# YaoTiancheng/DirectComputeRayTracing

Measured on AMD Instinct MI355X. Metric: Mrays/s and ms/spp at 1920x1080, 8-bounce wavefront, higher is better.
Workload: dtype f32; 1 GPU; cornell_box_obj 1920x1080, 1733 spp (1 spp/step, film stripes across 1 GPU(s)), 8 bounces, wavefront, point light; spp=1733, max_bounce=8, streams_per_gpu=3, snapshot_spp=1733, parallelism=single GPU, 3 concurrent pipelines per GPU (cost-balanced bands), partition=balanced, interleave=False, bands_per_rank=3, rays=48252902736

## Files before the change

### directcomputeraytracing_amd/_abi.py

```python
from __future__ import annotations

import ctypes as C
import os
from pathlib import Path

PKG_DIR = Path(__file__).resolve().parent
LIB_PATH = PKG_DIR / "libdcrt.so"

DCRT_OK = 0
ABI_VERSION = 4
ERRORS = {-1: "DCRT_E_INVALID_ARG", -2: "DCRT_E_HIP", -3: "DCRT_E_NO_SCENE", -4: "DCRT_E_IO",
          -5: "DCRT_E_LIMIT", -6: "DCRT_E_NO_DEVICE"}
LIGHT_INDEX_INVALID = 0xFFFFFFFF
FEATURE_GGX_SAMPLE_VNDF = 0x01
FEATURE_NO_FRONT_TO_BACK = 0x02
FEATURE_LIGHT_VISIBLE = 0x04
FEATURE_WATERTIGHT = 0x08
FEATURE_ALLOW_ANYHIT = 0x10
FEATURE_DEFAULT = FEATURE_GGX_SAMPLE_VNDF | FEATURE_LIGHT_VISIBLE | FEATURE_WATERTIGHT
FILTER_BOX, FILTER_TRIANGLE, FILTER_GAUSSIAN, FILTER_MITCHELL, FILTER_LANCZOS = range(5)
MATERIAL_DIFFUSE, MATERIAL_PLASTIC, MATERIAL_CONDUCTOR, MATERIAL_DIELECTRIC, MATERIAL_THIN_DIELECTRIC = range(5)
MAX_LIGHT_COUNT = 5000
DIRTY_LIGHTS = 0x01
DIRTY_MATERIALS = 0x02
DIRTY_INSTANCE_FLAGS = 0x04
DIRTY_CAMERA = 0x08
DIRTY_SCENE = 0x10
(OUTPUT_PATH_TRACING, OUTPUT_SHADING_NORMAL, OUTPUT_SHADING_TANGENT, OUTPUT_ALBEDO, OUTPUT_NEGATIVE_NDOTV,
 OUTPUT_BACKFACE, OUTPUT_ITERATION_COUNT) = range(7)


class Vertex(C.Structure):
    _fields_ = [("position", C.c_float * 3), ("normal", C.c_float * 3), ("tangent", C.c_float * 3),
                ("texcoord", C.c_float * 2)]


class BVHNode(C.Structure):
    _fields_ = [("bbox_min", C.c_float * 3), ("bbox_max", C.c_float * 3), ("right_child_or_prim_index", C.c_uint32),
                ("misc", C.c_uint32)]


class Material(C.Structure):
    _fields_ = [("albedo", C.c_float * 3), ("albedo_texture_index", C.c_int32), ("ior", C.c_float * 3),
# ... 91 lines not shown


class AdaptiveReport(C.Structure):
    _fields_ = [("images", C.c_uint32), ("check_points", C.c_uint32), ("pixel_samples", C.c_uint64),
                ("active_blocks", C.c_uint32), ("total_blocks", C.c_uint32)]


class RayStats(C.Structure):
    _fields_ = [("extension_rays", C.c_uint64), ("shadow_rays", C.c_uint64), ("new_paths", C.c_uint64),
                ("iterations", C.c_uint64), ("images_completed", C.c_uint64)]


class FilmPartition(C.Structure):
    _fields_ = [("world_size", C.c_uint32), ("rank", C.c_uint32), ("stripe_height", C.c_uint32),
                ("halo_rows", C.c_uint32)]


class TraversalStats(C.Structure):
    _fields_ = [("ext_node_visits", C.c_uint64), ("ext_triangle_tests", C.c_uint64), ("ext_blas_entries", C.c_uint64),
                ("shadow_node_visits", C.c_uint64), ("shadow_triangle_tests", C.c_uint64),
                ("shadow_blas_entries", C.c_uint64), ("ext_launches", C.c_uint64), ("ext_kernel_ms", C.c_double),
                ("ext_max_node_visits", C.c_uint64), ("shadow_max_node_visits", C.c_uint64),
                ("material_launches", C.c_uint64), ("material_kernel_ms", C.c_double),
                ("control_launches", C.c_uint64), ("control_kernel_ms", C.c_double)]


class TracerInfo(C.Structure):
    _fields_ = [("path_pool_size", C.c_uint32), ("scene_in_lds", C.c_uint32), ("cached_nodes", C.c_uint32),
                ("cached_triangles", C.c_uint32), ("cast_block", C.c_uint32), ("traversal_stack", C.c_uint32),
                ("material_generic", C.c_uint32), ("pair_traversal", C.c_uint32), ("control_grid", C.c_uint32),
                ("material_grid", C.c_uint32), ("cast_grid", C.c_uint32), ("material_lds", C.c_uint32),
                ("cast_identity", C.c_uint32), ("stack_lds_rows", C.c_uint32), ("ring_rows", C.c_uint32),
                ("cast_waves_per_cu", C.c_uint32), ("shadow_cells", C.c_uint32), ("shadow_cell_max_leaves", C.c_uint32),
                ("shadow_cell_mean_leaves", C.c_float), ("shadow_inline", C.c_uint32)]


class ShadowCellsInfo(C.Structure):
    _fields_ = [("resolution", C.c_uint32), ("leaf_count", C.c_uint32), ("node_count", C.c_uint32),
                ("max_leaves", C.c_uint32), ("mean_leaves", C.c_float), ("r0", C.c_float)]


class UploadStats(C.Structure):
    _fields_ = [("scene_uploads", C.c_uint64), ("material_updates", C.c_uint64), ("light_updates", C.c_uint64),
                ("instance_flag_updates", C.c_uint64), ("geometry_bytes", C.c_uint64), ("shading_bytes", C.c_uint64),
                ("graph_invalidations", C.c_uint64)]


class MaterialSetting(C.Structure):
    _fields_ = [("albedo", C.c_float * 3), ("roughness", C.c_float), ("ior", C.c_float * 3), ("opacity", C.c_float),
                ("k", C.c_float * 3), ("tiling", C.c_float * 2), ("material_type", C.c_uint32),
                ("albedo_texture_index", C.c_int32), ("opacity_texture_index", C.c_int32),
                ("internal_scattering_mode", C.c_uint32), ("multiscattering", C.c_uint32),
                ("is_two_sided", C.c_uint32), ("has_roughness_texture", C.c_uint32)]


class SceneSettings(C.Structure):
    _fields_ = [("resolution", C.c_uint32 * 2), ("max_bounce_count", C.c_uint32), ("camera_type", C.c_uint32),
                ("fov_x", C.c_float), ("focal_length", C.c_float), ("focal_distance", C.c_float),
                ("relative_aperture", C.c_float), ("aperture_blade_count", C.c_uint32), ("aperture_rotation", C.c_float),
                ("film_size", C.c_float * 2), ("camera_position", C.c_float * 3), ("camera_euler_angles", C.c_float * 3),
                ("features", C.c_uint32), ("has_environment_light", C.c_uint32), ("environment_color", C.c_float * 3),
                ("env_cube_rgb", C.POINTER(C.c_float)), ("env_cube_size", C.c_uint32),
                ("mesh_light_count", C.c_uint32), ("punctual_light_count", C.c_uint32),
                ("material_count", C.c_uint32), ("texture_count", C.c_uint32)]


class ObjMesh(C.Structure):
# ... 123 lines not shown
    ("dcrt_tracer_render_guides", _I, [_P, _U, _U]),
    ("dcrt_tracer_guide_device_ptrs", _I, [_P, C.POINTER(_P), C.POINTER(_P)]),
    ("dcrt_tracer_read_guides", _I, [_P, _FP, _FP]),
    ("dcrt_tracer_denoise", _I, [_P, C.POINTER(DenoiseParams)]),
    ("dcrt_tracer_denoise_device", _I, [_P, C.POINTER(DenoiseParams), _U, _U, _P, _P, _P, _P]),
    ("dcrt_tracer_denoise_images", _I, [_P, C.POINTER(DenoiseParams), _U, _U, _FP, _FP, _FP, _FP]),
    ("dcrt_tracer_read_denoised", _I, [_P, _FP]),
    ("dcrt_tracer_denoised_device_ptr", _I, [_P, C.POINTER(_P)]),
    ("dcrt_tracer_resolve_denoised", _I, [_P, C.POINTER(PostFxParams), C.POINTER(C.c_uint8), _FP]),
    ("dcrt_tracer_denoise_timings", _I, [_P, _FP, _U, C.POINTER(C.c_uint32)]),
    ("dcrt_tracer_set_convergence", _I, [_P, _I]),
    ("dcrt_tracer_film_image_count", _I, [_P, C.POINTER(C.c_uint32)]),
    ("dcrt_tracer_half_film_device_ptr", _I, [_P, C.POINTER(_P)]),
    ("dcrt_tracer_read_half_film", _I, [_P, _FP]),
    ("dcrt_tracer_add_half_film_device", _I, [_P, _P]),
    ("dcrt_tracer_noise", _I, [_P, C.c_float, C.POINTER(NoiseStats)]),
    ("dcrt_tracer_noise_device", _I, [_P, _U, _U, _P, _P, C.c_float, _P, _P, C.POINTER(NoiseStats)]),
    ("dcrt_tracer_film_pass_timing", _I, [_P, C.POINTER(C.c_uint64), C.POINTER(C.c_double)]),
    ("dcrt_tracer_noise_map_device_ptrs", _I, [_P, C.POINTER(_P), C.POINTER(_P)]),
    ("dcrt_tracer_read_noise_maps", _I, [_P, _FP, _FP]),
    ("dcrt_tracer_render_converged", _I, [_P, _U, C.POINTER(ConvergeParams), C.POINTER(FilterParams), C.POINTER(NoiseStats),
                                          C.POINTER(C.c_int)]),
    ("dcrt_tracer_set_adaptive", _I, [_P, _I]),
    ("dcrt_tracer_set_sample_blocks", _I, [_P, C.POINTER(C.c_uint32), _U]),
    ("dcrt_tracer_get_sample_blocks", _I, [_P, C.POINTER(C.c_uint32), _U, C.POINTER(C.c_uint32)]),
    ("dcrt_tracer_update_sample_blocks", _I, [_P, C.c_float, _U, C.POINTER(C.c_uint32)]),
    ("dcrt_tracer_sample_blocks_device", _I, [_P, _U, _U, _P, _P, C.c_float, _U, _P, _P, C.POINTER(C.c_uint32)]),
    ("dcrt_tracer_adaptive_timings", _I, [_P, _FP, _FP, _FP]),
    ("dcrt_tracer_render_adaptive", _I, [_P, _U, C.POINTER(ConvergeParams), _U, C.POINTER(FilterParams), C.POINTER(NoiseStats),
                                         C.POINTER(C.c_int), C.POINTER(AdaptiveReport)]),
    ("dcrt_write_bmp", _I, [C.c_char_p, _U, _U, C.POINTER(C.c_uint8)]),
    ("dcrt_device_math_eval", _I, [_P, _I, _FP, _U, _FP]),
    ("dcrt_device_bsdf_eval", _I, [_P, C.POINTER(BsdfProbeMaterial), _U, _FP, _FP, _U, _FP, _FP]),
    ("dcrt_device_bsdf_sample", _I, [_P, C.POINTER(BsdfProbeMaterial), _U, _FP, _FP, _U, _FP, _FP, _FP, C.POINTER(C.c_uint32)]),
]

_lib = None


class DCRTError(RuntimeError):
    pass


def load_library(path: os.PathLike | str | None = None):
    global _lib
    if _lib is not None:
        return _lib
    p = Path(path) if path else Path(os.environ.get("DCRT_LIB", LIB_PATH))
    if not p.exists():
        raise DCRTError(f"native library {p} is missing: run __graft_entry__.build() (no CPU fallback exists)")
    lib = C.CDLL(str(p))
    for name, res, args in SIGNATURES:
        fn = getattr(lib, name)
        fn.restype = res
        fn.argtypes = args
    if lib.dcrt_abi_version() != ABI_VERSION:
        raise DCRTError(f"{p}: ABI version {lib.dcrt_abi_version()}, this binding expects {ABI_VERSION}")
    _lib = lib
    return lib


def check(rc: int, what: str = "") -> None:
    if rc != DCRT_OK:
        lib = load_library()
        msg = lib.dcrt_last_error().decode(errors="replace")
        raise DCRTError(f"{what or 'dcrt call'} failed: {ERRORS.get(rc, rc)}: {msg}")
# ... 5 lines not shown
```

### directcomputeraytracing_amd/csrc/device/dbsdf.h

```cpp
#pragma once

#include "dscene.h"

namespace dcrt {
namespace dev {

struct LCtx { V3 H; float WOdotH; };
DEV void calc_h(V3 wo, V3 wi, LCtx& c)
{
    c.H = wi + wo;
    c.H = all_zero(c.H) ? mk(0.0f, 0.0f, 0.0f) : normalize(c.H);
    c.WOdotH = dot(c.H, wo);
}

DEV float fresnel_dielectric(float cosThetaI, float etaO, float etaI)
{
    cosThetaI = fminf(fmaxf(cosThetaI, -1.0f), 1.0f);
    if (cosThetaI < 0.0f) { const float t = etaO; etaO = etaI; etaI = t; cosThetaI = -cosThetaI; }
    const float sinThetaI = sqrtf(1.0f - cosThetaI * cosThetaI);
    const float sinThetaT = etaO / etaI * sinThetaI;
    if (sinThetaT >= 1.0f) return 1.0f;
    const float cosThetaT = sqrtf(1.0f - sinThetaT * sinThetaT);
    const float Rparl = ((etaI * cosThetaI) - (etaO * cosThetaT)) / ((etaI * cosThetaI) + (etaO * cosThetaT));
    const float Rperp = ((etaO * cosThetaI) - (etaI * cosThetaT)) / ((etaO * cosThetaI) + (etaI * cosThetaT));
// ... 184 lines not shown
DEV V3 specular_brdf_sample(V3 wo, float* value, float* pdf, LCtx& c)
{
    const V3 wi = mk(-wo.x, -wo.y, wo.z);
    c.H = mk(0.0f, 0.0f, 1.0f); c.WOdotH = wo.z;
    if (wo.z <= 0.0f) return wi;
    *value = 1.0f / wi.z;
    *pdf = 1.0f;
    return wi;
}
template <bool NO_SCALE>
DEV V3 specular_bsdf_sample(V3 wo, float sample, float etaO, float etaI, bool thin, float* value, float* pdf, LCtx& c)
{
    V3 wi = mk(0.0f, 0.0f, 0.0f);
    c.H = mk(0.0f, 0.0f, 1.0f); c.WOdotH = wo.z;
    if (etaO == etaI) { *value = 1.0f / wo.z; *pdf = 1.0f; return -wo; }
    if (wo.z == 0.0f) return wi;
    float F = fresnel_dielectric(wo.z, etaO, etaI);
    float T = 1.0f - F;
    if (thin && F < 1.0f) { F = F + T * T * F / (1.0f - F * F); T = 1.0f - F; }
    if (sample < F) {
        wi = mk(-wo.x, -wo.y, wo.z);
        *value = F / wi.z;
        *pdf = F;
    } else {
        wi = !thin ? refract(-wo, mk(0.0f, 0.0f, 1.0f), etaO / etaI) : -wo;
        if (wi.z == 0.0f) return wi;
        if (NO_SCALE) *value = T / (-wi.z);
        else *value = T * (!thin ? (etaO * etaO) / (etaI * etaI) : 1.0f) / (-wi.z);
        *pdf = T;
    }
    return wi;
}

DEV V3 isf_factor(const DeviceScene& s, float alpha, V3 albedo, float ior, uint32_t mode)
{
    if (mode == DCRT_INTERNAL_SCATTERING_IGNORE) return mk(1.0f, 1.0f, 1.0f);
    const float avg = lut_brdf_dielectric_avg(s, alpha, ior, true);
    const float f = 1.0f - avg;
    V3 factor = mk(f, f, f);
    if (mode == DCRT_INTERNAL_SCATTERING_MULTIPLE)
        factor = mk(factor.x / (1.0f - albedo.x * avg), factor.y / (1.0f - albedo.y * avg), factor.z / (1.0f - albedo.z * avg));
    return factor;
}
DEV V3 to_tbn(V3 w, V3 t, V3 b, V3 n) { return mk(dot(w, t), dot(w, b), dot(w, n)); }
DEV V3 from_tbn(V3 w, V3 t, V3 b, V3 n)
{
    return mk(w.x * t.x + w.y * b.x + w.z * n.x, w.x * t.y + w.y * b.y + w.z * n.y, w.x * t.z + w.y * b.z + w.z * n.z);
}
DEV V3 splat(float f) { return mk(f, f, f); }

struct DielectricMs { float E, Eavg, EinvAvg, ratio; };
DEV DielectricMs dielectric_ms(const DeviceScene& s, float cosThetaO, float alpha, float ior, bool inverted)
{
    const float EavgEnter = lut_bsdf_avg(s, alpha, ior, true);
    const float FavgEnter = favg_dielectric(1.0f / ior);
    const float EavgLeave = lut_bsdf_avg(s, alpha, ior, false);
    const float FavgLeave = favg_dielectric(ior);
    const float rf = reciprocal_factor(FavgLeave, FavgEnter, EavgLeave, EavgEnter, ior);
    DielectricMs d;
    d.E = lut_bsdf(s, cosThetaO, alpha, ior, inverted);
    const float Favg = inverted ? FavgEnter : FavgLeave;
    d.Eavg = inverted ? EavgEnter : EavgLeave;
    d.EinvAvg = inverted ? EavgLeave : EavgEnter;
    d.ratio = (inverted ? 1.0f - rf : rf) * (1.0f - Favg);
    return d;
}

struct BsdfFrame {
    V3 b, wo;
    bool inv;
    bool any;
    float E, Eavg;
    float diel;
    V3 isf;
    DielectricMs dms;
};
DEV BsdfFrame bsdf_frame(const DeviceScene& s, V3 woW, const Intersection& it)
{
    BsdfFrame f;
    f.b = cross(it.normal, it.tangent);
    f.wo = to_tbn(woW, it.tangent, f.b, it.normal);
    f.inv = f.wo.z < 0.0f;
    if (f.inv) f.wo.z = -f.wo.z;
    f.any = !f.inv || it.isTwoSided;
    const float cosO = f.wo.z;
    const uint32_t type = it.materialType;
    f.E = 0.0f; f.Eavg = 0.0f; f.diel = 0.0f; f.isf = mk(1.0f, 1.0f, 1.0f);
    f.dms.E = 0.0f; f.dms.Eavg = 0.0f; f.dms.EinvAvg = 0.0f; f.dms.ratio = 0.0f;
    if (it.multiscattering && (type == DCRT_MATERIAL_TYPE_PLASTIC || type == DCRT_MATERIAL_TYPE_CONDUCTOR) && f.any) {
        f.E = lut_brdf(s, cosO, it.alpha);
        f.Eavg = lut_brdf_avg(s, it.alpha);
    }
    if (type == DCRT_MATERIAL_TYPE_PLASTIC && f.any) {
        f.diel = lut_brdf_dielectric(s, cosO, it.alpha, it.ior.x, false);
        f.isf = isf_factor(s, it.alpha, it.albedo, it.ior.x, it.internalScatteringMode);
    }
    if (type == DCRT_MATERIAL_TYPE_DIELECTRIC && it.multiscattering && !(it.alpha < kAlphaThreshold))
        f.dms = dielectric_ms(s, cosO, it.alpha, it.ior.x, f.inv);
    return f;
}

DEV V3 evaluate_bsdf(const DeviceScene& s, bool vndf, V3 wiW, const BsdfFrame& f, const Intersection& it)
{
    const V3 wo = f.wo;
    V3 wi = to_tbn(wiW, it.tangent, f.b, it.normal);
    const bool inv = f.inv;
    if (inv) wi.z = -wi.z;
    LCtx c;
    calc_h(wo, wi, c);
    const bool smooth = it.alpha < kAlphaThreshold;
    V3 value = mk(0.0f, 0.0f, 0.0f);
    const uint32_t type = it.materialType;
    if (type != DCRT_MATERIAL_TYPE_DIELECTRIC && type != DCRT_MATERIAL_TYPE_THIN_DIELECTRIC) {
        bool hasL = false, hasCT = false, hasMS = false, dielF = false;
        float ratioL = 0.0f;
        const float E = f.E, Eavg = f.Eavg;
        V3 Fms = mk(0.0f, 0.0f, 0.0f), isf = mk(1.0f, 1.0f, 1.0f);
        const bool any = f.any;
        if (type == DCRT_MATERIAL_TYPE_DIFFUSE && any) {
            hasL = true; ratioL = 1.0f;
        } else if (type == DCRT_MATERIAL_TYPE_PLASTIC && any) {
            hasL = true; hasCT = !smooth; hasMS = it.multiscattering && !smooth; dielF = true;
            ratioL = 1.0f - f.diel;
            if (hasMS) {
                const float fm = ms_fresnel(Eavg, favg_dielectric(it.ior.x));
                Fms = splat(fm);
                ratioL = fmaxf(ratioL - Fms.x * (1.0f - E), 0.0f);
            }
// ... 191 lines not shown
```

### directcomputeraytracing_amd/csrc/device/dscene.h

```cpp
#pragma once

#include "../../../include/dcrt.h"
#include "dmath.h"
#include "../host/shadow_cells.h"

namespace dcrt {
namespace dev {

constexpr uint32_t kCapMatDiffuse = 1u << 0;
constexpr uint32_t kCapMatPlastic = 1u << 1;
constexpr uint32_t kCapMatConductor = 1u << 2;
constexpr uint32_t kCapMatDielectric = 1u << 3;
constexpr uint32_t kCapMatThin = 1u << 4;
constexpr uint32_t kCapMultiscatter = 1u << 5;
constexpr uint32_t kCapTextures = 1u << 6;
constexpr uint32_t kCapLightPoint = 1u << 7;
constexpr uint32_t kCapLightMesh = 1u << 8;
constexpr uint32_t kCapLightDirectional = 1u << 9;
constexpr uint32_t kCapLightEnv = 1u << 10;
constexpr uint32_t kCapEnvCube = 1u << 11;
constexpr uint32_t kCapAll = (1u << 12) - 1u;
constexpr uint32_t kCapMaterialsMask = 0x1Fu;
constexpr uint32_t kCapLightShift = 7;
constexpr uint32_t kCapOpaqueDelta = kCapMatDiffuse | kCapMatPlastic | kCapMatConductor | kCapLightPoint | kCapLightDirectional;
// ... 20 lines not shown
    const uint32_t* instanceFlags;
    const uint32_t* instanceIdentity;
    const uint32_t* overrides;
    const dcrt_material* materials;
    const dcrt_light* lights;
    const TextureDesc* textures;
    const uint8_t* texels;
    const float* srgbTable;
    const float* envCube;
    const uint16_t* lutBrdf;
    const uint16_t* lutBrdfAvg;
    const uint16_t* lutBrdfDielectric;
    const uint16_t* lutBrdfDielectricAvg;
    const uint16_t* lutBsdf;
    const uint16_t* lutBsdfAvg;
    uint32_t instanceCount;
    uint32_t nodeCount;
    uint32_t triangleCount;
    uint32_t envCubeSize;
    uint32_t stackSize;
    uint32_t stackRows;
    uint32_t ringRows;
    uint32_t* spill;
    uint32_t cachedNodes;
    uint32_t cachedTris;
    uint32_t cachedInstances;
    uint32_t singlePrimLeaves;
    uint32_t pairLayout;
    uint32_t skipRoot;
    uint32_t ldsMaterials, ldsLights;
    const uint64_t* shadowCells;
    const uint32_t* shadowLeaves;
    uint32_t shadowRes;
};

__host__ __device__ inline uint32_t material_lds_bytes(uint32_t T, uint32_t I, uint32_t M, uint32_t L)
{
    return 16u * (9u * T + 3u * I) + 4u * (2u * I + 13u * M + 7u * L);
}

__host__ __device__ inline uint32_t material_cells_lds_bytes(uint32_t nodes, uint32_t T) { return 32u * nodes + 144u * T + 4u * kCellWords; }
__host__ __device__ inline uint32_t material_cells_lds_offset(uint32_t shadingBytes) { return (shadingBytes + 15u) & ~15u; }

enum : int { kLayoutFlat = 0, kLayoutPairs = 1, kLayoutScene = 2 };
template <int LAYOUT>
DEV void node_children(const DeviceScene& sc, uint32_t node, uint32_t right, uint32_t* left, uint32_t* rightChild)
{
    const uint32_t r = right | (node & 0x80000000u);
    const bool pairs = LAYOUT == kLayoutPairs || (LAYOUT == kLayoutScene && sc.pairLayout != 0u);
    *left = pairs ? r : node + 1u;
    *rightChild = pairs ? r + 1u : r;
}


DEV float4* scene_cache(const DeviceScene& sc, uint32_t* stackMem, uint32_t shift)
{
    return (float4*)(stackMem + (sc.stackRows << shift));
}
typedef float LoadF4 __attribute__((ext_vector_type(4)));
DEV float4 lds_load4(const float4* genericLds, uint32_t i)
{
    const __attribute__((address_space(3))) LoadF4* p = (const __attribute__((address_space(3))) LoadF4*)(uint32_t)(uintptr_t)genericLds;
    const LoadF4 v = p[i];
    return make_float4(v.x, v.y, v.z, v.w);
}
DEV uint64_t global_load_u64(const uint64_t* g, size_t i)
{
// ... 657 lines not shown
    if (r > (float)(slices - 1)) return slices - 1;
    return (int)r;
}
DEV float remap(uint32_t dim, float u) { return u * ((float)(dim - 1) / (float)dim) + 0.5f / (float)dim; }
DEV float sample_array(const uint16_t* tex, uint32_t w, uint32_t h, uint32_t slices, float uu, float vv, float ww, uint32_t dz, uint32_t off)
{
    const float slicePos = ww * ((float)dz - 1.0f);
    const float fraction = slicePos - floorf(slicePos);
    const float u = remap(w, uu), v = remap(h, vv);
    const uint32_t s0 = (uint32_t)(int32_t)slicePos + off;
    const uint32_t s1 = (uint32_t)(int32_t)slicePos + 1u + off;
    const int i0 = array_slice((float)s0, (int)slices), i1 = array_slice((float)s1, (int)slices);
    const float a = bilinear_u16(tex + (size_t)i0 * w * h, (int)w, (int)h, u, v);
    const float b = bilinear_u16(tex + (size_t)i1 * w * h, (int)w, (int)h, u, v);
    return lerp(a, b, fraction);
}
DEV float lut_brdf(const DeviceScene& s, float cosThetaO, float alpha)
{
    return bilinear_u16(s.lutBrdf, 32, 32, remap(32, cosThetaO), remap(32, alpha));
}
DEV float lut_brdf_avg(const DeviceScene& s, float alpha)
{
    const float u = remap(32, alpha);
    return bilinear_u16(s.lutBrdfAvg, 32, 1, u, u);
}
DEV float lut_brdf_dielectric(const DeviceScene& s, float cosThetaO, float alpha, float eta, bool entering)
{
    return sample_array(s.lutBrdfDielectric, 32, 16, 32, cosThetaO, alpha, (eta - 1.0f) / 2.0f, 16, entering ? 16u : 0u);
}
DEV float lut_brdf_dielectric_avg(const DeviceScene& s, float alpha, float eta, bool entering)
{
    return sample_array(s.lutBrdfDielectricAvg, 16, 16, 2, alpha, (eta - 1.0f) / 2.0f, 0.0f, 1, entering ? 1u : 0u);
}
DEV float lut_bsdf(const DeviceScene& s, float cosThetaO, float alpha, float eta, bool entering)
{
    return sample_array(s.lutBsdf, 32, 16, 32, cosThetaO, alpha, (eta - 1.0f) / 2.0f, 16, entering ? 16u : 0u);
}
DEV float lut_bsdf_avg(const DeviceScene& s, float alpha, float eta, bool entering)
{
    return sample_array(s.lutBsdfAvg, 16, 16, 2, alpha, (eta - 1.0f) / 2.0f, 0.0f, 1, entering ? 1u : 0u);
}

DEV int wrapi(int i, int n) { const int r = i % n; return r < 0 ? r + n : r; }
DEV void texel(const DeviceScene& s, const TextureDesc& t, int x, int y, float* o)
{
    if (t.format == DCRT_TEXTURE_FORMAT_R8_UNORM) {
        o[0] = (float)s.texels[t.offset + (size_t)y * t.width + x] / 255.0f; o[1] = 0.0f; o[2] = 0.0f; o[3] = 1.0f;
    } else {
        const uint8_t* p = s.texels + t.offset + ((size_t)y * t.width + x) * 4;
        o[0] = s.srgbTable[p[0]]; o[1] = s.srgbTable[p[1]]; o[2] = s.srgbTable[p[2]]; o[3] = (float)p[3] / 255.0f;
    }
}
DEV void sample_texture_wrap(const DeviceScene& s, uint32_t index, float u, float v, float* out)
{
    const TextureDesc t = s.textures[index];
    if (t.width == 0 || t.height == 0) { out[0] = out[1] = out[2] = out[3] = 0.0f; return; }
    const int w = (int)t.width, h = (int)t.height;
    const float x = u * (float)w - 0.5f, y = v * (float)h - 0.5f;
    const float fx0 = floorf(x), fy0 = floorf(y);
    const float fx = x - fx0, fy = y - fy0;
    const int x0 = wrapi((int)fx0, w), x1 = wrapi((int)fx0 + 1, w);
    const int y0 = wrapi((int)fy0, h), y1 = wrapi((int)fy0 + 1, h);
    float a[4], b[4], c[4], d[4];
    texel(s, t, x0, y0, a); texel(s, t, x1, y0, b); texel(s, t, x0, y1, c); texel(s, t, x1, y1, d);
    for (int i = 0; i < 4; ++i) {
        const float top = a[i] * (1.0f - fx) + b[i] * fx;
// ... 2 lines not shown
    }
}
DEV V3 sample_env(const DeviceScene& s, V3 d)
{
    const float ax = fabsf(d.x), ay = fabsf(d.y), az = fabsf(d.z);
    int face; float sc, tc, ma;
    if (ax >= ay && ax >= az) { ma = ax; if (d.x >= 0.0f) { face = 0; sc = -d.z; tc = -d.y; } else { face = 1; sc = d.z; tc = -d.y; } }
    else if (ay >= az) { ma = ay; if (d.y >= 0.0f) { face = 2; sc = d.x; tc = d.z; } else { face = 3; sc = d.x; tc = -d.z; } }
    else { ma = az; if (d.z >= 0.0f) { face = 4; sc = d.x; tc = -d.y; } else { face = 5; sc = -d.x; tc = -d.y; } }
    const float u = (sc / ma + 1.0f) * 0.5f, v = (tc / ma + 1.0f) * 0.5f;
    const int n = (int)s.envCubeSize;
    const float x = u * (float)n - 0.5f, y = v * (float)n - 0.5f;
    const float fx0 = floorf(x), fy0 = floorf(y);
    const float fx = x - fx0, fy = y - fy0;
    const int x0 = clampi((int)fx0, 0, n - 1), x1 = clampi((int)fx0 + 1, 0, n - 1);
    const int y0 = clampi((int)fy0, 0, n - 1), y1 = clampi((int)fy0 + 1, 0, n - 1);
    const float* base = s.envCube + (size_t)face * n * n * 3;
    float o[3];
    for (int i = 0; i < 3; ++i) {
        const float a = base[((size_t)y0 * n + x0) * 3 + i], b = base[((size_t)y0 * n + x1) * 3 + i];
        const float c = base[((size_t)y1 * n + x0) * 3 + i], e = base[((size_t)y1 * n + x1) * 3 + i];
        const float top = a * (1.0f - fx) + b * fx;
        const float bot = c * (1.0f - fx) + e * fx;
        o[i] = top * (1.0f - fy) + bot * fy;
    }
    return mk(o[0], o[1], o[2]);
}

struct Intersection {
    V3 albedo; float alpha;
    V3 position, normal, tangent, geometryNormal, ior;
    bool isTwoSided, backface, multiscattering;
    uint32_t internalScatteringMode, materialType, lightIndex, triangleIndex;
};

DEV V3 bary3(V3 p0, V3 p1, V3 p2, float u, float v)
{
    V3 r1 = p1 - p0, r2 = p2 - p0;
    r1 = r1 * u; r2 = r2 * v;
    r1 = r1 + p0; r1 = r1 + r2;
    return r1;
}

template <uint32_t CAPS = kCapAll>
DEV void hit_to_intersection(const DeviceScene& s, const HitRecord& h, Intersection& it)
{
    const uint32_t inst = h.inst, tri = h.tri & 0x7FFFFFFFu;
    it.lightIndex = s.instanceLightIndices[inst];
    it.triangleIndex = tri;
    const uint32_t ov = s.overrides[inst];
    const float4* P = s.triVerts + (size_t)tri * 3;
    const float4* Q = s.triShade + (size_t)tri * 6;
    const float4 q0 = P[0], q1 = P[1], q2 = P[2];
    const float4 a0 = Q[0], b0 = Q[1], a1 = Q[2], b1 = Q[3], a2 = Q[4], b2 = Q[5];
    const float u = h.u, v = h.v;
    const V3 p0 = mk(q0.x, q0.y, q0.z), p1 = mk(q1.x, q1.y, q1.z), p2 = mk(q2.x, q2.y, q2.z);
    it.position = bary3(p0, p1, p2, u, v);
    it.normal = normalize(bary3(mk(a0.x, a0.y, a0.z), mk(a1.x, a1.y, a1.z), mk(a2.x, a2.y, a2.z), u, v));
    V3 tangent = bary3(mk(a0.w, b0.x, b0.y), mk(a1.w, b1.x, b1.y), mk(a2.w, b2.x, b2.y), u, v);
    float tl = length(tangent);
    if (tl >= 0.000001f) {
        tangent = tangent - it.normal * dot(tangent, it.normal);
        tl = length(tangent);
    }
    if (tl < 0.000001f) {
        tangent = cross(it.normal, mk(0.0f, 1.0f, 0.0f));
        tl = length(tangent);
        tangent = tl >= 0.000001f ? tangent : mk(1.0f, 0.0f, 0.0f);
    }
    it.tangent = tangent / tl;
    it.geometryNormal = normalize(cross(p2 - p0, p1 - p0));
    const uint32_t mid = ov != DCRT_INSTANCE_MATERIAL_OVERRIDE_NONE ? ov : __float_as_uint(q1.w);
    const dcrt_material& m = s.materials[mid];
    if constexpr ((CAPS & kCapTextures) == 0u) {
        __builtin_assume(m.albedo_texture_index == -1);
        __builtin_assume((m.flags & DCRT_MATERIAL_FLAG_ROUGHNESS_TEXTURE) == 0u);
    }
    if constexpr ((CAPS & kCapMultiscatter) == 0u) __builtin_assume((m.flags & DCRT_MATERIAL_FLAG_MULTISCATTERING) == 0u);
    if constexpr ((CAPS & kCapMaterialsMask) != kCapMaterialsMask) {
        __builtin_assume((m.flags & DCRT_MATERIAL_FLAG_TYPE_MASK) <= DCRT_MATERIAL_TYPE_THIN_DIELECTRIC);
        __builtin_assume(((CAPS >> (m.flags & DCRT_MATERIAL_FLAG_TYPE_MASK)) & 1u) != 0u);
    }
    float r1x = b1.z - b0.z, r1y = b1.w - b0.w;
    float r2x = b2.z - b0.z, r2y = b2.w - b0.w;
    r1x = r1x * u; r1y = r1y * u; r2x = r2x * v; r2y = r2y * v;
    r1x = r1x + b0.z; r1y = r1y + b0.w;
    float tcx = r1x + r2x, tcy = r1y + r2y;
    tcx = tcx * m.tex_tiling[0]; tcy = tcy * m.tex_tiling[1];
    V3 albedo = ld3(m.albedo);
    if (m.albedo_texture_index != -1) {
        float rgba[4];
        sample_texture_wrap(s, (uint32_t)m.albedo_texture_index, tcx, tcy, rgba);
        albedo = albedo * mk(rgba[0], rgba[1], rgba[2]);
    }
    const float checker = ((f2u_sat(tcx * 2.0f) + f2u_sat(tcy * 2.0f)) & 0x1u) != 0 ? 1.0f : 0.0f;
    float roughness = m.roughness;
    roughness = roughness * ((m.flags & DCRT_MATERIAL_FLAG_ROUGHNESS_TEXTURE) != 0 ? checker : 1.0f);
    it.albedo = albedo;
    it.alpha = roughness * roughness;
    it.ior = ld3(m.ior);
    it.materialType = m.flags & DCRT_MATERIAL_FLAG_TYPE_MASK;
    it.isTwoSided = (m.flags & DCRT_MATERIAL_FLAG_IS_TWOSIDED) != 0;
    it.multiscattering = (m.flags & DCRT_MATERIAL_FLAG_MULTISCATTERING) != 0;
    it.internalScatteringMode = (m.flags & DCRT_MATERIAL_FLAG_INTERNAL_SCATTERING_MASK) >> DCRT_MATERIAL_FLAG_INTERNAL_SCATTERING_SHIFT;
    it.backface = (h.tri & 0x80000000u) != 0;
    const float4* M = s.transforms + (size_t)inst * 3;
    it.position = mul43(it.position, 1.0f, M);
    it.normal = normalize(mul43(it.normal, 0.0f, M));
    it.geometryNormal = normalize(mul43(it.geometryNormal, 0.0f, M));
    it.tangent = normalize(mul43(it.tangent, 0.0f, M));
}

struct LightSample {
    V3 radiance, wi;
    float pdf, distance;
    bool isDelta;
};
DEV V3 tri_pos(const DeviceScene& s, uint32_t tri, int k)
{
    const float4 q = s.triVerts[(size_t)tri * 3 + k];
    return mk(q.x, q.y, q.z);
}

template <uint32_t CAPS = kCapAll>
DEV LightSample sample_light(const DeviceScene& s, V3 p, uint32_t lightCount, Rng& rng)
{
    LightSample r;
    r.radiance = mk(0.0f, 0.0f, 0.0f); r.wi = mk(0.0f, 0.0f, 0.0f); r.pdf = 0.0f; r.distance = 0.0f; r.isDelta = false;
    const float sel = next1(rng);
    const uint32_t li = (uint32_t)floorf(sel * (float)lightCount);
    const dcrt_light& L = s.lights[li];
    assume_light_caps<CAPS>(L.flags);
    if constexpr ((CAPS & kCapEnvCube) == 0u) __builtin_assume(s.envCube == nullptr);
    if (L.flags & DCRT_LIGHT_FLAGS_POINT_LIGHT) {
        r.wi = ld3(L.position_or_triangle_range) - p;
        r.distance = length(r.wi);
        r.wi = r.wi / r.distance;
        r.radiance = ld3(L.radiance) / (r.distance * r.distance);
        r.pdf = 1.0f;
        r.isDelta = true;
    } else if (L.flags & DCRT_LIGHT_FLAGS_DIRECTIONAL_LIGHT) {
        r.wi = -ld3(L.position_or_triangle_range);
        r.distance = inf();
// ... 69 lines not shown
```

### directcomputeraytracing_amd/csrc/device/kernels_impl.h

```cpp
#include "kernels.h"

namespace dcrt {
namespace dev {

#ifdef DCRT_PHASE_CLOCKS
__device__ unsigned long long g_phaseClk[24];
#define DCRT_PHASE_INIT unsigned long long clk_[6] = {0, 0, 0, 0, 0, 0}; unsigned long long tP_ = __builtin_amdgcn_s_memtime()
#define DCRT_PHASE(i) do { const unsigned long long t_ = __builtin_amdgcn_s_memtime(); clk_[i] += t_ - tP_; tP_ = t_; } while (0)
#define DCRT_PHASE_COUNT(i) (++clk_[i])
#define DCRT_PHASE_FLUSH() do { if ((threadIdx.x & 63u) == 0) for (int i_ = 0; i_ < 6; ++i_) atomicAdd(&g_phaseClk[i_], clk_[i_]); } while (0)
#define DCRT_MCLK_INIT unsigned long long mclk_[8] = {0, 0, 0, 0, 0, 0, 0, 0}; unsigned long long mT_ = __builtin_amdgcn_s_memtime()
#define DCRT_MCLK(i) do { const unsigned long long t_ = __builtin_amdgcn_s_memtime(); mclk_[i] += t_ - mT_; mT_ = t_; } while (0)
#define DCRT_MCLK_FLUSH(items) do { mclk_[7] += (items); if ((threadIdx.x & 63u) == 0) for (int i_ = 0; i_ < 8; ++i_) atomicAdd(&g_phaseClk[8 + i_], mclk_[i_]); } while (0)
#define DCRT_MCLK_PARAMS , unsigned long long (&mclk_)[8], unsigned long long& mT_
#define DCRT_MCLK_ARGS , mclk_, mT_
#else
#define DCRT_MCLK_PARAMS
#define DCRT_MCLK_ARGS
#define DCRT_MCLK_INIT do {} while (0)
#define DCRT_MCLK(i) do {} while (0)
#define DCRT_MCLK_FLUSH(items) do {} while (0)
#define DCRT_PHASE_INIT do {} while (0)
#define DCRT_PHASE(i) do {} while (0)
#define DCRT_PHASE_COUNT(i) do {} while (0)
// ... 74 lines not shown
__global__ void set_idle_kernel(PathPool pool, Counters* counters, Globals* g, uint32_t totalBlocks)
{
    const uint32_t tid = blockIdx.x * blockDim.x + threadIdx.x;
    if (tid < pool.size) pool.flags[tid] = kFlagIdle;
    if (tid < 2 * (uint32_t)(sizeof(Counters) / 4)) ((uint32_t*)counters)[tid] = 0u;
    if (tid < kShards) g->nextBlock[tid * kShardStride] = 0u;
    if (tid == 0) {
        g->totalBlocks = totalBlocks;
        g->batchImages = 1u;
        g->batchCap = 1u;
        g->imageComplete = 0u;
        g->poolIdle = 0u;
        g->prevLive = 0u;
        g->stopped = 0u;
        g->imagesDone = 0u;
        g->imageTarget = 1u;
        g->staticFill = 0u;
        g->staticGrid = 0u;
        g->skipFilm = 0u;
    }
}

__device__ __forceinline__ void begin_batch_claims(Globals* g)
{
    const uint32_t G = g->staticGrid, wavesPerGroup = kControlBlock >> 6;
    for (uint32_t s = 0; s < kShards; ++s) {
        const uint32_t blocks = g->totalBlocks > s ? (g->totalBlocks - s + kShards - 1) / kShards : 0u;
        const uint32_t waves = G > s ? ((G - s + kShards - 1) / kShards) * wavesPerGroup : 0u;
        g->nextBlock[s * kShardStride] = G ? min(blocks, waves) : 0u;
    }
    g->staticFill = G ? 1u : 0u;
}

__global__ void build_tri_verts_kernel(const dcrt_vertex* vertices, const uint32_t* triangles, const uint32_t* materialIds,
                                       uint32_t count, float4* out, float4* shade)
{
    const uint32_t t = blockIdx.x * blockDim.x + threadIdx.x;
    if (t >= count) return;
    V3 p[3];
    for (int k = 0; k < 3; ++k) {
        const dcrt_vertex& v = vertices[triangles[t * 3 + k]];
        p[k] = mk(v.position[0], v.position[1], v.position[2]);
        shade[(size_t)t * 6 + 2 * k] = make_float4(v.normal[0], v.normal[1], v.normal[2], v.tangent[0]);
        shade[(size_t)t * 6 + 2 * k + 1] = make_float4(v.tangent[1], v.tangent[2], v.texcoord[0], v.texcoord[1]);
    }
    const V3 cp = cross(p[1] - p[0], p[2] - p[0]);
    const float degenerate = dot(cp, cp) == 0.0f ? 1.0f : 0.0f;
    out[(size_t)t * 3] = make_float4(p[0].x, p[0].y, p[0].z, degenerate);
    out[(size_t)t * 3 + 1] = make_float4(p[1].x, p[1].y, p[1].z, __uint_as_float(materialIds[t]));
    out[(size_t)t * 3 + 2] = make_float4(p[2].x, p[2].y, p[2].z, 0.0f);
}

__global__ __launch_bounds__(kControlBlock) void control_kernel(PathPool pool, Film film, const FrameConstants* __restrict__ fc, Counters* cnt,
                                                       const Counters* prev, Globals* g, uint32_t debugRng)
{
    __shared__ uint32_t sm[64];
    if (g->stopped) return;
    {
        QueueMapN<kFinShards> fm;
        qmap(prev, kQFinish, &fm);
        const uint32_t nFin = drained(prev) ? 0u : fm.prefix[kFinShards];
        for (uint32_t i = blockIdx.x * blockDim.x + threadIdx.x; i < nFin; i += gridDim.x * blockDim.x) {
            const uint32_t f = qpos(pool.finCap, fm, i);
            const FinishRec fr = pool.finPrevRec[f];
            const bool shadowHit = pool.finHitPrev[f] != 0u;
            const uint32_t path = asu(fr.lsrSlot.z);
// ... 57 lines not shown
    bool newPath = false;
    V3 o = mk(0.0f, 0.0f, 0.0f), d = mk(0.0f, 0.0f, 0.0f);
    Rng rng;
    rng.s0 = rng.s1 = rng.s2 = rng.s3 = 0u;
    if (got) {
        uint32_t px = 0, py = 0, image = 0;
        if (block_pixel(*fc, film, block, lane, &px, &py, &image)) {
            rng = rng_init(px, py, image_seed(*fc, image));
            const float psx = next1(rng), psy = next1(rng);
            const float fsx = (psx + (float)px) / (float)fc->resolution[0];
            const float fsy = (psy + (float)py) / (float)fc->resolution[1];
            const float a0 = next1(rng), a1 = next1(rng), a2 = next1(rng);
            generate_ray(*fc, fsx, fsy, a0, a1, a2, &o, &d);
            if (fc->features & DCRT_FEATURE_ALLOW_ANYHIT) pool.extOpacity[tid] = next1(rng);
            pool.pixel[tid] = image * (film.width * film.height) + py * film.width + px;
            pool.flags[tid] = 0u;
            newPath = true;
        }
    }
    uint32_t eslot, unused;
    block_append2(newPath, qctr(cnt, kQExt, shard), false, qctr(cnt, kQExt, shard), sm + 32, &eslot, &unused);
    if (newPath) {
        const uint32_t q = shard * pool.recCap + eslot;
        float4* r = ext_rec(pool.extRec, q);
        r[0] = make_float4(o.x, o.y, o.z, 0.0f);
        r[1] = make_float4(d.x, d.y, d.z, asf(tid));
        PathStateA& st = state_at(pool.stateA, q);
        st.rng = make_uint4(rng.s0, rng.s1, rng.s2, rng.s3);
        st.lsrMisc = make_float4(0.0f, 0.0f, asf(kFlagDelta | kFlagFirst), asf(tid));
    }
    }
}

template <uint32_t CAPS>
__device__ __forceinline__ void shade_path(const DeviceScene& sc, const FrameConstants& fc, const HitRecord& hit, V3 dir, Rng& rng,
                                           uint32_t& flags, float4& thr, const F3& li, V3& T, V3& L, V3& lsr, bool& terminate,
                                           bool& hasShadow, V3& nO, V3& nD, float4& sO, V3& sD, float& extOpacity,
                                           float& shadowOpacity DCRT_MCLK_PARAMS)
{
    const uint32_t bounce = flags & 0xFFu;
    const uint32_t features = fc.features;
    const bool vndf = (features & DCRT_FEATURE_GGX_SAMPLE_VNDF) != 0;
    const bool hasHit = hit.t != inf();
    Intersection it;
    it.lightIndex = DCRT_LIGHT_INDEX_INVALID; it.triangleIndex = 0;
    it.geometryNormal = mk(0.0f, 0.0f, 0.0f);
    if (hasHit) hit_to_intersection<CAPS>(sc, hit, it);
    DCRT_MCLK(1);
    T = mk(thr.x, thr.y, thr.z);
    L = mk(li.x, li.y, li.z);
    {
        const uint32_t lightIndex = hasHit ? it.lightIndex : fc.envLightIndex;
        const bool visible = (features & DCRT_FEATURE_LIGHT_VISIBLE) != 0;
        if (visible ? lightIndex != DCRT_LIGHT_INDEX_INVALID : (bounce > 0 && lightIndex != DCRT_LIGHT_INDEX_INVALID)) {
            V3 radiance; float lightPdf;
            evaluate_light<CAPS>(sc, lightIndex, it.triangleIndex, it.geometryNormal, dir, hit.t, fc.lightCount, &radiance, &lightPdf);
            if (lightPdf > 0.0f) {
                const float weight = !(flags & kFlagDelta) ? power_heuristic(thr.w, lightPdf) : 1.0f;
                L = L + T * radiance * weight;
            }
        }
    }
    lsr = mk(0.0f, 0.0f, 0.0f);
    if (bounce > fc.maxBounce || !hasHit) {
        flags |= kFlagTerminate;
        terminate = true;
    } else {
        const V3 wo = -dir;
        const BsdfFrame bf = bsdf_frame(sc, wo, it);
        if (fc.lightCount != 0) {
            const LightSample ls = sample_light<CAPS>(sc, it.position, fc.lightCount, rng);
            if (any_pos(ls.radiance) && ls.pdf > 0.0f) {
                const V3 bsdf = evaluate_bsdf(sc, vndf, ls.wi, bf, it);
                const float NdotWI = fabsf(dot(it.normal, ls.wi));
                const float bsdfPdf = evaluate_bsdf_pdf(sc, vndf, ls.wi, bf, it);
                const float weight = ls.isDelta ? 1.0f : power_heuristic(ls.pdf, bsdfPdf);
                lsr = T * ls.radiance * bsdf * NdotWI * weight / ls.pdf;
                const V3 so = offset_ray_origin(it.position, it.geometryNormal, ls.wi);
                sO = make_float4(so.x, so.y, so.z, ls.distance);
                sD = ls.wi;
                hasShadow = true;
            }
        }
        DCRT_MCLK(3);
        float bsdfPdf = 0.0f;
        bool isDelta = false;
        {
            const float sel = next1(rng);
            const float sx = next1(rng), sy = next1(rng);
            V3 wi, bsdf;
            sample_bsdf(sc, vndf, bf, sx, sy, sel, it, &wi, &bsdf, &bsdfPdf, &isDelta);
            if ((bsdf.x != 0.0f || bsdf.y != 0.0f || bsdf.z != 0.0f) && bsdfPdf != 0.0f) {
                const float NdotWI = fabsf(dot(it.normal, wi));
                T = T * bsdf * NdotWI / bsdfPdf;
                nO = offset_ray_origin(it.position, it.geometryNormal, wi);
                nD = wi;
                flags = (flags & 0xFFFFFF00u) | ((bounce + 1) & 0xFFu);
            } else {
                flags |= kFlagTerminate;
                terminate = true;
            }
        }
        thr.w = bsdfPdf;
        flags = isDelta ? flags | kFlagDelta : flags & ~kFlagDelta;
        if (features & DCRT_FEATURE_ALLOW_ANYHIT) {
            if (!terminate) extOpacity = next1(rng);
            if (hasShadow) shadowOpacity = next1(rng);
        }
// ... 14 lines not shown
template <uint32_t CAPS, int SCENE_LDS, bool PROBE = false, bool FUSED = false>
__global__ __launch_bounds__(DCRT_MATERIAL_BLOCK) DCRT_MATERIAL_OCCUPANCY void material_kernel(PathPool pool, DeviceScene sc, const FrameConstants* __restrict__ fcr, Counters* cnt,
                                                                             const Counters* prev, const SampleOut* __restrict__ sampleOut, ShadowInline si)
{
    static_assert(!FUSED || (SCENE_LDS == 1 && !PROBE), "FUSED: beside the whole LDS shading copy");
#if defined(DCRT_MATERIAL_PRIO) && DCRT_MATERIAL_PRIO > 0
    __builtin_amdgcn_s_setprio(DCRT_MATERIAL_PRIO);
#endif
    __shared__ uint32_t sm[96 + (FUSED ? 1 : 0)];
    QueueMap qm;
    qmap(prev, kQExt, &qm);
    const uint32_t virt = virtual_items(prev);
    const uint32_t count = drained(prev) ? 0u : (virt ? virt : qm.prefix[kShards]);
    const uint32_t shard = blockIdx.x % kShards;
    const uint32_t fshard = blockIdx.x % kFinShards;
    const FrameConstants& fcv = *fcr;
    const float4* cellNodes = nullptr;
    const float4* cellTris = nullptr;
    const uint32_t* cellLeaves = nullptr;
    uint32_t& inlineTotal = sm[FUSED ? 96 : 0];
    uint32_t inlineRays = 0;
    if constexpr (SCENE_LDS != 0) {
        extern __shared__ float4 sceneLds[];
        if (blockIdx.x * blockDim.x >= count) return;
        const uint32_t T = SCENE_LDS == 1 ? sc.triangleCount : 0u, I = sc.instanceCount;
        float4* tv = sceneLds;
        float4* ts = tv + 3u * T;
        float4* tf = ts + 6u * T;
        uint32_t* w = (uint32_t*)(tf + 3u * I);
        uint32_t* li = w;
        uint32_t* ov = li + I;
        uint32_t* mt = ov + I;
        uint32_t* lt = mt + 13u * sc.ldsMaterials;
        for (uint32_t i = threadIdx.x; i < 3u * T; i += blockDim.x) tv[i] = sc.triVerts[i];
        for (uint32_t i = threadIdx.x; i < 6u * T; i += blockDim.x) ts[i] = sc.triShade[i];
        for (uint32_t i = threadIdx.x; i < 3u * I; i += blockDim.x) tf[i] = sc.transforms[i];
        for (uint32_t i = threadIdx.x; i < I; i += blockDim.x) { li[i] = sc.instanceLightIndices[i]; ov[i] = sc.overrides[i]; }
        for (uint32_t i = threadIdx.x; i < 13u * sc.ldsMaterials; i += blockDim.x) mt[i] = ((const uint32_t*)sc.materials)[i];
        for (uint32_t i = threadIdx.x; i < 7u * sc.ldsLights; i += blockDim.x) lt[i] = ((const uint32_t*)sc.lights)[i];
        if constexpr (FUSED) {
            float4* cn = sceneLds + (material_cells_lds_offset(material_lds_bytes(T, I, sc.ldsMaterials, sc.ldsLights)) >> 4);
            float4* ct = cn + 2u * si.nodeCount;
            uint32_t* cl = (uint32_t*)(ct + kRotTriFloat4 * T);
            for (uint32_t i = threadIdx.x; i < 2u * si.nodeCount; i += blockDim.x) cn[i] = si.nodes[i];
            for (uint32_t i = threadIdx.x; i < kRotTriFloat4 * T; i += blockDim.x) ct[i] = rot_tri_float4(sc.triVerts, i);
            for (uint32_t i = threadIdx.x; i < kCellWords; i += blockDim.x) cl[i] = si.leaves[i];
            if (threadIdx.x == 0) inlineTotal = 0u;
            cellNodes = cn;
            cellTris = ct;
            cellLeaves = cl;
        }
        __syncthreads();
        if constexpr (SCENE_LDS == 1) {
            sc.triVerts = tv;
            sc.triShade = ts;
        }
        sc.transforms = tf;
        sc.instanceLightIndices = li;
        sc.overrides = ov;
        sc.materials = (const dcrt_material*)mt;
        sc.lights = (const dcrt_light*)lt;
    }
    DCRT_MCLK_INIT;
    uint32_t itemsDone = 0;
    uint32_t round = 0;
    for (uint32_t base = blockIdx.x * blockDim.x; base < count; base += gridDim.x * blockDim.x) {
    const uint32_t i = base + threadIdx.x;
    bool active = i < count;
    uint32_t newPixel = kNoPixel;
    if (virt && active) {
        newPixel = slot(pool.pixel, i);
        active = newPixel != kNoPixel;
    }
    bool terminate = false, hasShadow = false, ends = false;
    uint32_t path = 0, pix = 0;
    float4 sample = make_float4(0.0f, 0.0f, 0.0f, 0.0f);
    float2* outPos = nullptr;
    float4* outVal = nullptr;
    V3 nO = mk(0.0f, 0.0f, 0.0f), nD = mk(0.0f, 0.0f, 0.0f);
    float4 sO = make_float4(0.0f, 0.0f, 0.0f, 0.0f);
    V3 sD = mk(0.0f, 0.0f, 0.0f);
    uint32_t pathFlags = 0;
    float4 sThr = make_float4(0.0f, 0.0f, 0.0f, 0.0f);
    V3 sT = mk(0.0f, 0.0f, 0.0f), sL = mk(0.0f, 0.0f, 0.0f), sLsr = mk(0.0f, 0.0f, 0.0f);
    uint4 sRng = make_uint4(0u, 0u, 0u, 0u);
    if (active) {
        ++itemsDone;
        const float4 h4 = pool.hit[2 * i], hd = pool.hit[2 * i + 1];
        HitRecord hit;
        hit.t = h4.x; hit.u = h4.y; hit.v = h4.z; hit.tri = asu(h4.w); hit.inst = asu(hd.w);
        const V3 dir = mk(hd.x, hd.y, hd.z);
        Rng rng;
        uint32_t flags;
        float4 thr, l4, l2;
// ... 10 lines not shown
            const uint32_t q = qpos(pool.recCap, qm, i);
            const PathStateA& ps = state_at(pool.stateAPrev, q);
            const PathStateB& psB = state_at(pool.stateBPrev, q);
            const uint4 r4 = ps.rng;
            l2 = ps.lsrMisc;
            const float4 bThr = psB.thr, bLi = psB.liLsr;
            uint32_t shRaw = 0u;
            if constexpr (FUSED) {
                if (__ballot((asu(l2.z) & kFlagShadowPending) != 0u) != 0ull) shRaw = pool.shadowHitPrev[q];
            } else {
                shRaw = pool.shadowHitPrev[q];
            }
            rng.s0 = r4.x; rng.s1 = r4.y; rng.s2 = r4.z; rng.s3 = r4.w;
            path = asu(l2.w);
            flags = asu(l2.z);
            const bool first = (flags & kFlagFirst) != 0u;
            thr = first ? make_float4(1.0f, 1.0f, 1.0f, 0.0f) : bThr;
            l4 = first ? make_float4(0.0f, 0.0f, 0.0f, 0.0f) : bLi;
            shadowHit = (flags & kFlagShadowResolved) != 0u || ((flags & kFlagShadowPending) != 0u && shRaw != 0u);
            flags &= ~(kFlagFirst | kFlagShadowPending | kFlagShadowResolved);
        }
        F3 li{l4.x, l4.y, l4.z};
        {
            const F3 lsr0{l4.w, l2.x, l2.y};
            li.x = li.x + (!shadowHit ? lsr0.x : 0.0f);
            li.y = li.y + (!shadowHit ? lsr0.y : 0.0f);
            li.z = li.z + (!shadowHit ? lsr0.z : 0.0f);
        }
        uint32_t out = path;
        asm volatile("" : "+v"(out));
        float extOpacity = 0.0f, shadowOpacity = 0.0f;
        V3 T, L, lsr;
        DCRT_MCLK(0);
        shade_path<CAPS>(sc, fcv, hit, dir, rng, flags, thr, li, T, L, lsr, terminate, hasShadow, nO, nD, sO, sD,
                         extOpacity, shadowOpacity DCRT_MCLK_ARGS);
        DCRT_MCLK(4);
        if (fcv.features & DCRT_FEATURE_ALLOW_ANYHIT) {
            if (!terminate) slot(pool.extOpacity, out) = extOpacity;
            if (hasShadow) slot(pool.shadowOpacity, out) = shadowOpacity;
        }
        ends = terminate && !hasShadow;
        if constexpr (PROBE) {
            uint32_t* rowRays = sampleOut->rowRays;
            const uint32_t p = virt ? newPixel : slot(pool.pixel, out);
            const uint32_t W = fcv.resolution[0], wh = W * fcv.resolution[1];
            atomicAdd(&rowRays[(p % wh) / W], hasShadow ? 2u : 1u);
        }
        pathFlags = flags;
        sThr = thr;
        sT = T;
        sL = L;
        sLsr = lsr;
        sRng = make_uint4(rng.s0, rng.s1, rng.s2, rng.s3);
        if (ends || terminate) {
            const SampleOut so = *sampleOut;
            if (ends || so.debugRng) pix = slot(pool.pixel, out);
            if (ends) {
                sample = make_float4(L.x + 0.0f, L.y + 0.0f, L.z + 0.0f, 0.0f);
                outPos = so.samplePosition;
                outVal = so.sampleValue;
            }
            if (so.debugRng) sample_at(so.debugRng, pix) = make_uint4(rng.s0, rng.s1, rng.s2, rng.s3);
        }
    }
    bool inlined = false, occluded = false;
    if constexpr (FUSED) {
        const V3 sInv = inv_dir(sD);
// ... 821 lines not shown

__global__ __launch_bounds__(256) void cells_occlusion_kernel(DeviceScene sc, const dcrt_ray* rays, uint32_t n, uint32_t features,
                                                               uint32_t* occluded)
{
    extern __shared__ uint32_t stackMem[];
    uint32_t* leafWords = (uint32_t*)(scene_cache(sc, stackMem, block_shift()) + sc.cachedNodes * 2u + sc.cachedTris * kRotTriFloat4);
    if (threadIdx.x < kCellWords) leafWords[threadIdx.x] = sc.shadowLeaves[threadIdx.x];
    scene_cache_load<true>(sc, stackMem, block_shift());
    const bool watertight = (features & DCRT_FEATURE_WATERTIGHT) != 0;
    for (uint32_t i = blockIdx.x * blockDim.x + threadIdx.x; i < n; i += gridDim.x * blockDim.x) {
        const dcrt_ray r = rays[i];
        const bool occ = cells_occluded(sc, make_float4(r.origin[0], r.origin[1], r.origin[2], r.t_max),
                                        make_float4(r.direction[0], r.direction[1], r.direction[2], 0.0f), watertight,
                                        stackMem + threadIdx.x, block_shift(), leafWords);
        occluded[i] = occ ? 1u : 0u;
    }
}

__global__ void math_eval_kernel(int function, const float* x, uint32_t n, float* y)
{
    const uint32_t i = blockIdx.x * blockDim.x + threadIdx.x;
    if (i >= n) return;
    switch (function) {
    case 0: y[i] = det_sin(x[i]); break;
    case 1: y[i] = det_cos(x[i]); break;
    case 2: y[i] = det_exp(x[i]); break;
    case 4: y[i] = det_log(x[i]); break;
    case 5: y[i] = rcp_ieee(x[i]); break;
    case 6: y[i] = 1.0f / x[i]; break;
    default: y[i] = det_atan(x[i]); break;
    }
}

__device__ __forceinline__ Intersection bsdf_probe_intersection(const dcrt_bsdf_probe_material& m)
{
    Intersection it;
    it.albedo = mk(m.albedo[0], m.albedo[1], m.albedo[2]);
    it.alpha = m.alpha;
    it.position = mk(0.0f, 0.0f, 0.0f);
    it.normal = mk(0.0f, 0.0f, 1.0f);
    it.tangent = mk(1.0f, 0.0f, 0.0f);
    it.geometryNormal = mk(0.0f, 0.0f, 1.0f);
    it.ior = mk(m.ior[0], m.ior[1], m.ior[2]);
    it.isTwoSided = m.two_sided != 0;
    it.backface = false;
    it.multiscattering = m.multiscattering != 0;
    it.internalScatteringMode = m.internal_scattering_mode;
    it.materialType = m.type;
    it.lightIndex = DCRT_LIGHT_INDEX_INVALID;
    it.triangleIndex = 0;
    return it;
}
__global__ void bsdf_eval_kernel(DeviceScene sc, dcrt_bsdf_probe_material m, uint32_t features, const float* wi, const float* wo,
                                 uint32_t n, float* f, float* pdf)
{
    const uint32_t i = blockIdx.x * blockDim.x + threadIdx.x;
    if (i >= n) return;
    const bool vndf = (features & DCRT_FEATURE_GGX_SAMPLE_VNDF) != 0;
    const Intersection it = bsdf_probe_intersection(m);
    const V3 a = mk(wi[3 * i], wi[3 * i + 1], wi[3 * i + 2]), b = mk(wo[3 * i], wo[3 * i + 1], wo[3 * i + 2]);
    const BsdfFrame bf = bsdf_frame(sc, b, it);
    const V3 v = evaluate_bsdf(sc, vndf, a, bf, it);
    f[3 * i] = v.x; f[3 * i + 1] = v.y; f[3 * i + 2] = v.z;
    pdf[i] = evaluate_bsdf_pdf(sc, vndf, a, bf, it);
}
__global__ void bsdf_sample_kernel(DeviceScene sc, dcrt_bsdf_probe_material m, uint32_t features, const float* wo, const float* u,
                                   uint32_t n, float* wi, float* f, float* pdf, uint32_t* delta)
{
    const uint32_t i = blockIdx.x * blockDim.x + threadIdx.x;
    if (i >= n) return;
    const bool vndf = (features & DCRT_FEATURE_GGX_SAMPLE_VNDF) != 0;
    const Intersection it = bsdf_probe_intersection(m);
    const V3 b = mk(wo[3 * i], wo[3 * i + 1], wo[3 * i + 2]);
    const BsdfFrame bf = bsdf_frame(sc, b, it);
    V3 w, v; float p; bool d;
    sample_bsdf(sc, vndf, bf, u[3 * i], u[3 * i + 1], u[3 * i + 2], it, &w, &v, &p, &d);
    wi[3 * i] = w.x; wi[3 * i + 1] = w.y; wi[3 * i + 2] = w.z;
    f[3 * i] = v.x; f[3 * i + 1] = v.y; f[3 * i + 2] = v.z;
    pdf[i] = p;
    delta[i] = d ? 1u : 0u;
}

struct FilterConsts { float radius, gaussianAlpha, gaussianExp, mf[7]; uint32_t tau, kind; };

__device__ __forceinline__ float filter_1d_sinc(float x) { x = fabsf(x); return x >= 1e-5f ? det_sin(3.1415926535f * x) / (3.1415926535f * x) : 1.0f; }
__device__ __forceinline__ float evaluate_filter(const FilterConsts& c, float px, float py)
{
    const float r = c.radius;
    switch (c.kind) {
    case DCRT_FILTER_TRIANGLE: return fmaxf(0.0f, r - fabsf(px)) * fmaxf(0.0f, r - fabsf(py));
    case DCRT_FILTER_GAUSSIAN: {
        const float gx = fmaxf(0.0f, det_exp(-c.gaussianAlpha * px * px) - c.gaussianExp);
        const float gy = fmaxf(0.0f, det_exp(-c.gaussianAlpha * py * py) - c.gaussianExp);
        return gx * gy;
    }
    case DCRT_FILTER_MITCHELL: {
        float v[2] = { px / c.radius, py / c.radius }, o[2];
        for (int k = 0; k < 2; ++k) {
            const float x = fabsf(2.0f * v[k]);
            float m = x < 1.0f ? c.mf[4] * x * x * x + c.mf[5] * x * x + c.mf[6]
                               : (x < 2.0f ? c.mf[0] * x * x * x + c.mf[1] * x * x + c.mf[2] * x + c.mf[3] : 0.0f);
            o[k] = m * (1.0f / 6.0f);
        }
        return o[0] * o[1];
    }
// ... 816 lines not shown
```

### directcomputeraytracing_amd/csrc/device/tracer.hip

```cpp
#include <hip/hip_runtime.h>
#include <hip/hip_ext.h>

#include <dlfcn.h>

#include <algorithm>
#include <cmath>
#include <cstdio>
#include <cstdlib>
#include <cstring>
#include <map>
#include <mutex>
#include <string>
#include <type_traits>
#include <limits>
#include <vector>

#include "../../../include/dcrt.h"
#include "../host/bvh_layout.h"
#include "../host/film_rows.h"
#include "kernels_impl.h"

namespace dcrt {
void SetLastError(const std::string& s);
int CheckFilterParams(const dcrt_filter_params& f);
// ... 198 lines not shown
    bool ldsTrim = true;
    bool flatCast = true;
    bool flatMerge = true;
    uint32_t shadowCells = dcrt::kCellDefaultRes;
    int castBlocksPerCU = 0;
    int castGridMul = 0;
};
UploadKnobs ReadUploadKnobs()
{
    UploadKnobs k;
    k.castBlock = (uint32_t)EnvInt("DCRT_CAST_BLOCK", 0);
    k.noLdsCache = EnvFlag("DCRT_NO_LDS_CACHE", false);
    if (std::getenv("DCRT_PAIR_TRAVERSAL")) k.pairTraversal = EnvFlag("DCRT_PAIR_TRAVERSAL", false) ? 1 : 0;
    k.topNodes = (uint32_t)EnvInt("DCRT_TOP_NODES", (int)k.topNodes);
    k.nodeQuads = EnvFlag("DCRT_NODE_QUADS", true);
    k.identCast = EnvFlag("DCRT_IDENT_CAST", true);
    k.stackRing = EnvInt("DCRT_STACK_RING", -1);
    if (std::getenv("DCRT_CAST_LDS_RESERVE")) k.castLdsReserve = (size_t)std::max(0, EnvInt("DCRT_CAST_LDS_RESERVE", 0));
    k.skipRoot = (uint32_t)std::max(0, std::min(16, EnvInt("DCRT_SKIP_ROOT", (int)k.skipRoot)));
    k.ldsTrim = EnvFlag("DCRT_LDS_TRIM", true);
    k.flatCast = EnvFlag("DCRT_FLAT_CAST", true);
    k.flatMerge = EnvFlag("DCRT_FLAT_MERGE", true);
    k.shadowCells = (uint32_t)std::max(0, std::min((int)dcrt::kCellMaxRes, EnvInt("DCRT_SHADOW_CELLS", (int)k.shadowCells)));
    k.castBlocksPerCU = EnvInt("DCRT_CAST_BLOCKS_PER_CU", 0);
    k.castGridMul = EnvInt("DCRT_CAST_GRID_MUL", 0);
    return k;
}

struct ShadingKnobs {
    bool materialGeneric = false;
    uint32_t materialLds = 16384;
    bool materialLdsPartial = true;
    uint32_t fusedShadow = 1;
};
ShadingKnobs ReadShadingKnobs()
{
    ShadingKnobs k;
    k.materialGeneric = EnvFlag("DCRT_MATERIAL_GENERIC", false);
    k.materialLds = (uint32_t)std::max(0, EnvInt("DCRT_MATERIAL_LDS", (int)k.materialLds));
    k.materialLdsPartial = EnvFlag("DCRT_MATERIAL_LDS_PARTIAL", true);
    k.fusedShadow = (uint32_t)std::max(0, EnvInt("DCRT_FUSED_SHADOW", (int)k.fusedShadow));
    return k;
}

size_t g_ldsPerCU = 163840;
constexpr size_t kLdsGranule = 1280;
int LdsResident(size_t lds, const void* kernel = nullptr)
{
    if (kernel) {
        hipFuncAttributes attr{};
        if (hipFuncGetAttributes(&attr, kernel) == hipSuccess) lds += attr.sharedSizeBytes;
    }
    return lds ? (int)(g_ldsPerCU / ((lds + kLdsGranule - 1) / kLdsGranule * kLdsGranule)) : 1 << 20;
}

struct CastLaunch {
    CastFn kernel;
    size_t lds;
    const DeviceScene& scene;
    uint32_t resident;
};

struct CastPlan {
    uint32_t block = 256;
    uint32_t perCU = 0;
    bool allCached = false;
    bool pair = false;
    bool ident = false;
    bool flat = false;
    uint32_t ringRows = 0;
    uint32_t cellsRes = 0;
    size_t ldsWholeStack = 0;
    size_t ldsRing = 0;
    size_t ldsFlat = 0;
// ... 21 lines not shown
    uint32_t cuCount = 1;
    CreateKnobs knobs;
    uint32_t iterationsPerRender = kDefaultIterations;
    bool debugRng = false;
    int mode = 0;
    dcrt_output_params output{ DCRT_OUTPUT_PATH_TRACING, 20u };

    uint32_t poolSize = 0;
    uint32_t controlGrid = 0, materialGrid = 0;
    std::vector<void*> poolAllocs;
    PathPool pool{};
    float4* extRecs = nullptr;
    PathStateA* stateRecsA = nullptr;
    PathStateB* stateRecsB = nullptr;
    uint32_t* shadowHits = nullptr;
    FinishRec* finRecs = nullptr;
    uint32_t* finHits = nullptr;
    FrameConstants* dFrame = nullptr;
    Counters* dCounters = nullptr;
    Globals* dGlobals = nullptr;
    Counters* hCounters = nullptr;
    dcrt_bxdf_luts* dLuts = nullptr;

    std::vector<void*> sceneAllocs;
    bool hasScene = false;
    CastPlan plan;
    dcrt_upload_stats uploadStats{};
    uint32_t sceneCaps = kCapAll;
    uint32_t materialCaps = kCapAll;
    uint32_t materialLds = 0;
    uint32_t materialLdsMode = 0;
    uint32_t fusedLds = 0;
    uint32_t fusedMask = 0;
    bool FusedShadow() const
    {
        return fusedLds != 0u && !rowProbe && plan.Cells(instrCounters, (frame.features & DCRT_FEATURE_ALLOW_ANYHIT) != 0);
    }
    dcrt_material* dMaterials = nullptr;
    dcrt_light* dLights = nullptr;
    uint32_t* dInstanceFlags = nullptr;
    std::vector<dcrt_material> hostMaterials;
    std::vector<dcrt_light> hostLights;
    uint64_t* dCells = nullptr;
    uint32_t* dCellLeaves = nullptr;
    ShadowCells cells;
    std::vector<dcrt_bvh_node> cellNodes;
    std::vector<dcrt_vertex> cellVertices;
    std::vector<uint32_t> cellTriangles;
    std::vector<dcrt_float4x3> cellTransforms;
    uint32_t megaResident = 0;
    uint32_t viewResident = 0;
    uint32_t viewResidentOpacity = 0;
    uint32_t drainResident = 0;

    std::vector<void*> filmAllocs, sampleAllocs, rowAllocs;
    Film film{};
    uint32_t filmW = 0, filmH = 0;
    uint32_t rowCount = 0;
    uint32_t bandCount = 0;
    dcrt_film_partition partition{ 1, 0, 64, 0 };
    std::vector<uint32_t> bands;
    uint32_t sampleImages = 0;
    uint32_t batchImages = 0;
    uint32_t lastSlot = 0;
    uint32_t seedStride = 1;
    bool keptSlots = false;
// ... 60 lines not shown
    bool adaptive = false;
    std::vector<void*> adaptiveAllocs, maskAllocs;
    uint32_t* dBlockFlags = nullptr;
    uint32_t* dBlockList = nullptr;
    uint32_t* dMaskCount = nullptr;
    uint32_t* dMaskFlags = nullptr;
    uint32_t maskFlagCap = 0;
    uint32_t blockTotal = 0;
    uint32_t listCount = 0;
    uint32_t listPixels = 0;
    bool inactiveFilled = false;
    bool listFrame = false;
    uint64_t pathsSkipped = 0;
    hipEvent_t adEvents[5] = {};
    bool adMaskTimed = false, adFillTimed = false;
    int AdaptiveEvents()
    {
        for (hipEvent_t& e : adEvents)
            if (!e) HIPCHECK(hipEventCreate(&e));
        return DCRT_OK;
    }

    ~dcrt_tracer();
    int Create(const dcrt_tracer_config& cfg);
    int BuildLuts();
    int UploadScene(const dcrt_flat_scene& s);
    int UploadArrays(const dcrt_flat_scene& s, std::vector<uint32_t>* identity);
    int PlanCast(const dcrt_flat_scene& s, const UploadKnobs& k, const std::vector<uint32_t>& identity);
    int PlanFlatCast(const dcrt_flat_scene& s, const UploadKnobs& k);
    int SizeGrids(const UploadKnobs& k);
    int CastOccupancy(CastFn k, size_t lds, int* out);
    void DeriveShading();
    int DeriveFusedShadow();
    int DeriveDrainGrid();
    int RederiveShading();
    int UpdateMaterials(const dcrt_material* materials, uint32_t count);
    int UpdateLights(const dcrt_light* lights, uint32_t count);
    int UpdateInstanceFlags(const uint32_t* flags, uint32_t count);
    int RebuildShadowCells();
    int CheckFrameLights() const;
    int SetFrame(const dcrt_frame_params& p);
    int SetPartition(const dcrt_film_partition& p);
    int SetBands(const uint32_t* b, uint32_t count, uint32_t halo);
    int EnsureFilm(uint32_t w, uint32_t h);
    int BuildRows();
    int UploadSampleOut();
    int SetRowProbe(bool on);
    int EnsureSamples(uint32_t images);
    int UploadFilter(const dcrt_filter_params& f);
    int ClearFilm();
    int LaunchFilm(uint32_t images, const Globals* guard, const float2* const* posList, const float4* const* valList,
                   uint32_t firstIndex);
    int AccumulateImages(const void* const* pos, const void* const* val, uint32_t count, const dcrt_filter_params& filter);
    int Accumulate(const dcrt_filter_params& filter);
    uint32_t AutoBatch(uint32_t count) const;
    int BeginImage();
    int LaunchIteration(uint32_t par, bool timed, bool sequenced);
    int LaunchGraph(bool sequenced, uint32_t iters);
    int BuildGraph(bool sequenced, uint32_t iters);
    int PrepareImages(uint32_t count);
    int RunIterations(uint32_t n);
    int ReadCompletion(bool* complete);
    int Render(uint32_t maxIterations);
    int LaunchView();
    int LaunchView(uint32_t type, const Film& target);
    int RenderImages(uint32_t firstSeed, uint32_t count, const dcrt_filter_params& filter, uint32_t stride = 1,
// ... 252 lines not shown
    const bool counts = scene.triangleCount > 0 && scene.triangleCount < (1u << 20) && scene.instanceCount < (1u << 20) &&
                        materialCount < (1u << 20) && lightCount < (1u << 20);
    const uint64_t whole = material_lds_bytes(scene.triangleCount, scene.instanceCount, materialCount, lightCount);
    const uint64_t rest = material_lds_bytes(0u, scene.instanceCount, materialCount, lightCount);
    materialLdsMode = !counts ? 0u : whole <= k.materialLds ? 1u : (k.materialLdsPartial && rest <= k.materialLds ? 2u : 0u);
    materialLds = materialLdsMode == 1 ? (uint32_t)whole : materialLdsMode == 2 ? (uint32_t)rest : 0u;
    for (DeviceScene* d : { &plan.scene, &plan.sceneFlat, &plan.sceneRing }) {
        d->ldsMaterials = materialLdsMode ? materialCount : 0u;
        d->ldsLights = materialLdsMode ? lightCount : 0u;
    }
}

int dcrt_tracer::DeriveFusedShadow()
{
    const ShadingKnobs k = ReadShadingKnobs();
    fusedLds = 0;
    fusedMask = k.fusedShadow > 1u ? k.fusedShadow - 1u : 0u;
    if (!k.fusedShadow || !plan.flat || !plan.cellsRes || materialLdsMode != 1u) return DCRT_OK;
    const uint32_t extra = material_cells_lds_bytes(plan.sceneFlat.cachedNodes, plan.scene.triangleCount);
    if (extra > k.materialLds) return DCRT_OK;
    const bool od = materialCaps == kCapOpaqueDelta;
    const void* plain = od ? (const void*)material_kernel<kCapOpaqueDelta, 1> : (const void*)material_kernel<kCapAll, 1>;
    const void* fused = od ? (const void*)material_kernel<kCapOpaqueDelta, 1, false, true> : (const void*)material_kernel<kCapAll, 1, false, true>;
    const size_t fusedBytes = material_cells_lds_offset(materialLds) + extra;
    int plainPerCU = 0, fusedPerCU = 0;
    HIPCHECK(hipOccupancyMaxActiveBlocksPerMultiprocessor(&plainPerCU, plain, (int)kMaterialBlock, materialLds));
    HIPCHECK(hipOccupancyMaxActiveBlocksPerMultiprocessor(&fusedPerCU, fused, (int)kMaterialBlock, fusedBytes));
    plainPerCU = std::min(plainPerCU, LdsResident(materialLds, plain));
    fusedPerCU = std::min(fusedPerCU, LdsResident(fusedBytes, fused));
    if (fusedPerCU >= plainPerCU && fusedPerCU > 0) fusedLds = extra;
    return DCRT_OK;
}

int dcrt_tracer::DeriveDrainGrid()
{
    const void* fn = materialCaps == kCapOpaqueDelta ? (const void*)drain_kernel<kCapOpaqueDelta> : (const void*)drain_kernel<kCapAll>;
    int drainPerCU = 0;
    HIPCHECK(hipOccupancyMaxActiveBlocksPerMultiprocessor(&drainPerCU, materialCaps == kCapOpaqueDelta ? drain_kernel<kCapOpaqueDelta> : drain_kernel<kCapAll>,
                                                          (int)plan.block, plan.ldsWholeStack));
    drainResident = (uint32_t)std::max(1, std::min(drainPerCU, LdsResident(plan.ldsWholeStack, fn))) * cuCount;
    return DCRT_OK;
}

int dcrt_tracer::RederiveShading()
{
    const uint32_t caps = materialCaps, mode = materialLdsMode, lds = materialLds, grid = drainResident;
    const uint32_t ldsM = plan.scene.ldsMaterials, ldsL = plan.scene.ldsLights;
    const uint32_t fused = fusedLds, mask = fusedMask;
    DeriveShading();
    CHECKED(DeriveFusedShadow());
    if (materialCaps != caps) CHECKED(DeriveDrainGrid());
    if (fusedMask != mask) newImage = true;
    if (materialCaps != caps || materialLdsMode != mode || materialLds != lds || drainResident != grid || fusedLds != fused ||
        plan.scene.ldsMaterials != ldsM || plan.scene.ldsLights != ldsL) {
        HIPCHECK(hipStreamSynchronize(stream));
        InvalidateGraph();
    }
    return DCRT_OK;
}

int dcrt_tracer::UpdateMaterials(const dcrt_material* materials, uint32_t count)
{
    Annotation an("UpdateMaterials");
    if (!hasScene) { SetLastError("no scene uploaded"); return DCRT_E_NO_SCENE; }
    CHECKED(ValidateMaterials(materials, count));
    if (count != hostMaterials.size()) { SetLastError("material count differs from the uploaded scene's"); return DCRT_E_INVALID_ARG; }
    HIPCHECK(hipStreamSynchronize(stream));
    hostMaterials.assign(materials, materials + count);
    HIPCHECK(hipMemcpyAsync(dMaterials, hostMaterials.data(), (size_t)count * sizeof(dcrt_material), hipMemcpyHostToDevice, stream));
    uploadStats.shading_bytes += (uint64_t)count * sizeof(dcrt_material);
    ++uploadStats.material_updates;
    CHECKED(RederiveShading());
    HIPCHECK(hipStreamSynchronize(stream));
    return DCRT_OK;
}

int dcrt_tracer::UpdateLights(const dcrt_light* lights, uint32_t count)
{
    Annotation an("UpdateLights");
    if (!hasScene) { SetLastError("no scene uploaded"); return DCRT_E_NO_SCENE; }
    CHECKED(ValidateLights(lights, count));
    HIPCHECK(hipStreamSynchronize(stream));
    if (count) hostLights.assign(lights, lights + count);
    else hostLights.clear();
    if (count) HIPCHECK(hipMemcpyAsync(dLights, hostLights.data(), (size_t)count * sizeof(dcrt_light), hipMemcpyHostToDevice, stream));
    uploadStats.shading_bytes += (uint64_t)count * sizeof(dcrt_light);
// ... 34 lines not shown
    dcrt::BuildShadowCells(cellNodes.data(), cellNodes.size(), s, plan.cellsRes, &cells);
    const uint32_t before = sceneFlat.shadowRes;
    HIPCHECK(hipStreamSynchronize(stream));
    if (cells.resolution) {
        HIPCHECK(hipMemcpyAsync(dCells, cells.cells.data(), cells.cells.size() * sizeof(uint64_t), hipMemcpyHostToDevice, stream));
        HIPCHECK(hipMemcpyAsync(dCellLeaves, cells.leafWords.data(), dcrt::kCellWords * sizeof(uint32_t), hipMemcpyHostToDevice, stream));
        HIPCHECK(hipStreamSynchronize(stream));
    }
    sceneFlat.shadowCells = cells.resolution ? dCells : nullptr;
    sceneFlat.shadowLeaves = cells.resolution ? dCellLeaves : nullptr;
    sceneFlat.shadowRes = cells.resolution;
    if (before != sceneFlat.shadowRes) InvalidateGraph();
    return DCRT_OK;
}

int dcrt_tracer::CheckFrameLights() const
{
    if (hasScene && frame.light_count > hostLights.size()) {
        SetLastError("frame light_count " + std::to_string(frame.light_count) + " exceeds the " + std::to_string(hostLights.size()) +
                     " lights uploaded");
        return DCRT_E_INVALID_ARG;
    }
    return DCRT_OK;
}

int dcrt_tracer::UploadScene(const dcrt_flat_scene& s)
{
    Annotation an("UploadScene");
    const UploadKnobs k = ReadUploadKnobs();
    std::vector<uint32_t> identity;
    CHECKED(UploadArrays(s, &identity));
    CHECKED(PlanCast(s, k, identity));
    CHECKED(SizeGrids(k));
    CHECKED(RebuildShadowCells());
    HIPCHECK(hipStreamSynchronize(stream));
    hasScene = true;
    newImage = true;
    return DCRT_OK;
}

int dcrt_tracer::UploadArrays(const dcrt_flat_scene& s, std::vector<uint32_t>* identity)
{
    if (!s.vertices || !s.triangles || !s.bvh_nodes || !s.material_ids || !s.instance_transforms ||
        !s.instance_light_indices || !s.instance_material_overrides || s.triangle_count == 0 ||
        s.bvh_node_count == 0 || s.instance_count == 0 || ValidateMaterials(s.materials, s.material_count) != DCRT_OK ||
        ValidateInstanceFlags(s.instance_flags, s.instance_count) != DCRT_OK) {
        SetLastError("incomplete flat scene");
        return DCRT_E_INVALID_ARG;
    }
    CHECKED(ValidateLights(s.lights, s.light_count));
    HIPCHECK(hipStreamSynchronize(stream));
    InvalidateGraph();
    FreeAll(&sceneAllocs);
    hasScene = false;
    ++uploadStats.scene_uploads;
    DeviceScene d{};
    uint64_t* const geometry = &uploadStats.geometry_bytes;
    uint64_t* const shading = &uploadStats.shading_bytes;
    dcrt_vertex* vtx = nullptr;
    uint32_t* tris = nullptr;
    dcrt_float4x3* xf = nullptr;
    CHECKED(Upload(&vtx, s.vertices, s.vertex_count, geometry));
    CHECKED(Upload(&tris, s.triangles, (size_t)s.triangle_count * 3, geometry));
    uint32_t stackNeed = 0;
    if (!dcrt::RequiredTraversalStack(s, &stackNeed)) { SetLastError("malformed BVH node references"); return DCRT_E_INVALID_ARG; }
    if (s.bvh_traversal_stack_size < stackNeed) {
        SetLastError("bvh_traversal_stack_size " + std::to_string(s.bvh_traversal_stack_size) +
                     " is below the uploaded BVH's depth " + std::to_string(stackNeed));
        return DCRT_E_INVALID_ARG;
    }
    uint32_t* mids = nullptr; uint32_t* lidx = nullptr; uint32_t* iflags = nullptr; uint32_t* ovr = nullptr;
    dcrt_material* mats = nullptr; dcrt_light* lights = nullptr;
    CHECKED(Upload(&mids, s.material_ids, s.triangle_count, geometry));
    CHECKED(Upload(&xf, s.instance_transforms, (size_t)s.instance_count * 2, geometry));
    CHECKED(Upload(&lidx, s.instance_light_indices, s.instance_count, geometry));
    CHECKED(Upload(&iflags, s.instance_flags, s.instance_count, shading));
    CHECKED(Upload(&ovr, s.instance_material_overrides, s.instance_count, geometry));
    *identity = dcrt::IdentityInstances(s);
    uint32_t* ident = nullptr;
    CHECKED(Upload(&ident, (const uint32_t*)identity->data(), s.instance_count, geometry));
    CHECKED(Upload(&mats, s.materials, s.material_count, shading));
    CHECKED(Upload(&lights, s.lights, s.light_count, shading, DCRT_MAX_LIGHT_COUNT));
    dMaterials = mats;
    dLights = lights;
    dInstanceFlags = iflags;
    hostMaterials.assign(s.materials, s.materials + s.material_count);
    if (s.light_count) hostLights.assign(s.lights, s.lights + s.light_count);
    else hostLights.clear();
    float4* triVerts = nullptr;
    float4* triShade = nullptr;
    CHECKED(DeviceAlloc(&triVerts, (size_t)s.triangle_count * 3, &sceneAllocs));
    CHECKED(DeviceAlloc(&triShade, (size_t)s.triangle_count * 6, &sceneAllocs));
    if (s.triangle_count)
        hipLaunchKernelGGL(build_tri_verts_kernel, dim3((s.triangle_count + 255) / 256), dim3(256), 0, stream, vtx, tris, mids,
                           s.triangle_count, triVerts, triShade);
    HIPCHECK(hipGetLastError());
    std::vector<TextureDesc> descs(std::max<uint32_t>(s.texture_count, 1));
    std::vector<uint8_t> blob;
    for (uint32_t i = 0; i < s.texture_count; ++i) {
        const dcrt_texture& t = s.textures[i];
        TextureDesc& td = descs[i];
        const size_t bpp = t.format == DCRT_TEXTURE_FORMAT_R8_UNORM ? 1 : 4;
        td.width = t.pixels ? t.width : 0; td.height = t.pixels ? t.height : 0; td.format = t.format;
        td.offset = (uint32_t)blob.size();
        if (t.pixels) blob.insert(blob.end(), t.pixels, t.pixels + (size_t)t.width * t.height * bpp);
        while (blob.size() % 4) blob.push_back(0);
    }
    if (blob.empty()) blob.resize(4, 0);
    TextureDesc* dDescs = nullptr; uint8_t* dBlob = nullptr; float* dSrgb = nullptr;
    CHECKED(Upload(&dDescs, (const TextureDesc*)descs.data(), descs.size(), geometry));
    CHECKED(Upload(&dBlob, (const uint8_t*)blob.data(), blob.size(), geometry));
    float srgb[256];
    for (int i = 0; i < 256; ++i) {
        const double c = i / 255.0;
        srgb[i] = (float)(c <= 0.04045 ? c / 12.92 : std::pow((c + 0.055) / 1.055, 2.4));
    }
    CHECKED(Upload(&dSrgb, (const float*)srgb, 256, geometry));
    float* dEnv = nullptr;
    if (s.env_cube_rgb && s.env_cube_size) CHECKED(Upload(&dEnv, s.env_cube_rgb, (size_t)6 * s.env_cube_size * s.env_cube_size * 3, geometry));
    d.triVerts = triVerts;
    d.triShade = triShade;
    d.vertices = vtx;
    d.triangles = tris;
    d.materialIds = mids;
    d.transforms = (const float4*)xf;
    d.instanceLightIndices = lidx;
    d.instanceFlags = iflags;
    d.instanceIdentity = ident;
    d.overrides = ovr;
// ... 465 lines not shown
int dcrt_tracer::LaunchIteration(uint32_t par, bool timed, bool sequenced)
{
    Annotation an("Iteration", !capturing);
    Counters* cnt = dCounters + par;
    Counters* next = dCounters + (par ^ 1u);
    PathPool pool = this->pool;
    pool.extRec = extRecs + (size_t)par * kShards * pool.recCap * 2;
    pool.extPrevRec = extRecs + (size_t)(par ^ 1u) * kShards * pool.recCap * 2;
    pool.stateA = stateRecsA + (size_t)par * kShards * pool.recCap;
    pool.stateB = stateRecsB + (size_t)par * kShards * pool.recCap;
    pool.stateAPrev = stateRecsA + (size_t)(par ^ 1u) * kShards * pool.recCap;
    pool.stateBPrev = stateRecsB + (size_t)(par ^ 1u) * kShards * pool.recCap;
    pool.shadowHit = shadowHits + (size_t)par * kShards * pool.recCap;
    pool.shadowHitPrev = shadowHits + (size_t)(par ^ 1u) * kShards * pool.recCap;
    pool.finRec = finRecs + (size_t)par * kFinShards * pool.finCap;
    pool.finPrevRec = finRecs + (size_t)(par ^ 1u) * kFinShards * pool.finCap;
    pool.finHit = finHits + (size_t)par * kFinShards * pool.finCap;
    pool.finHitPrev = finHits + (size_t)(par ^ 1u) * kFinShards * pool.finCap;
    const bool opacity = (frame.features & DCRT_FEATURE_ALLOW_ANYHIT) != 0;
    const CastLaunch cast = plan.Launch(instrCounters, opacity);
    const uint32_t castBlock = plan.block, castGrid = std::min<uint32_t>((poolSize + castBlock - 1) / castBlock, cast.resident);
    hipEvent_t c0 = nullptr, c1 = nullptr, m0 = nullptr, m1 = nullptr, e0 = nullptr, e1 = nullptr;
    if (timed) CHECKED(TimedPair(kTimedControl, &c0, &c1));
    {
        Annotation a("Control", !capturing);
        Film claims = film;
        claims.blockList = sequenced && adaptive ? dBlockList : nullptr;
        hipExtLaunchKernelGGL(control_kernel, dim3(controlGrid), dim3(kControlBlock), 0, stream, c0, c1, 0, pool, claims,
                              (const FrameConstants*)dFrame, cnt, (const Counters*)next, dGlobals, (uint32_t)(film.debugRng != nullptr));
    }
    const bool fused = FusedShadow();
    ShadowInline si{};
    if (fused) si = ShadowInline{ plan.sceneFlat.nodes, plan.sceneFlat.shadowCells, plan.sceneFlat.shadowLeaves, plan.sceneFlat.cachedNodes, plan.sceneFlat.shadowRes };
    const uint32_t materialBytes = rowProbe ? 0u : fused ? material_cells_lds_offset(materialLds) + fusedLds : materialLds;
    auto material = rowProbe ? material_kernel<kCapAll, 0, true>
                  : fused ? (materialCaps == kCapOpaqueDelta ? material_kernel<kCapOpaqueDelta, 1, false, true> : material_kernel<kCapAll, 1, false, true>)
                  : materialCaps == kCapOpaqueDelta
                        ? (materialLdsMode == 1 ? material_kernel<kCapOpaqueDelta, 1>
                                                : materialLdsMode == 2 ? material_kernel<kCapOpaqueDelta, 2> : material_kernel<kCapOpaqueDelta, 0>)
                        : (materialLdsMode == 1 ? material_kernel<kCapAll, 1>
                                                : materialLdsMode == 2 ? material_kernel<kCapAll, 2> : material_kernel<kCapAll, 0>);
    if (timed) CHECKED(TimedPair(kTimedMaterial, &m0, &m1));
    {
        Annotation a("Material", !capturing);
        hipExtLaunchKernelGGL(material, dim3(materialGrid), dim3(kMaterialBlock), materialBytes, stream, m0, m1, 0, pool, plan.scene,
                              (const FrameConstants*)dFrame, cnt, (const Counters*)next, (const SampleOut*)dSampleOut, si);
    }
    if (timed) CHECKED(TimedPair(kTimedCast, &e0, &e1));
    Annotation castAnnotation(knobs.mergedCasts ? "Extension + shadow ray cast" : "Extension ray cast, shadow ray cast", !capturing);
    if (knobs.mergedCasts) {
        hipExtLaunchKernelGGL(cast.kernel, dim3(castGrid), dim3(castBlock), cast.lds, stream, e0, e1, 0, pool, cast.scene,
                              (const FrameConstants*)dFrame, cnt, next, dGlobals, dInstr);
    } else {
        auto ext = instrCounters ? (opacity ? extension_kernel<true, true> : extension_kernel<true, false>)
                                 : (opacity ? extension_kernel<false, true> : extension_kernel<false, false>);
        auto shadow = instrCounters ? (opacity ? shadow_kernel<true, true> : shadow_kernel<true, false>)
                                    : (opacity ? shadow_kernel<false, true> : shadow_kernel<false, false>);
        hipExtLaunchKernelGGL(ext, dim3(castGrid), dim3(castBlock), cast.lds, stream, e0, e1, 0, pool, cast.scene,
                              (const FrameConstants*)dFrame, (const Counters*)cnt, dGlobals, dInstr);
        hipLaunchKernelGGL(shadow, dim3(castGrid), dim3(castBlock), cast.lds, stream, pool, cast.scene, (const FrameConstants*)dFrame, cnt,
                           next, dGlobals, dInstr);
    }
    if (knobs.drainPaths) {
        auto drain = materialCaps == kCapOpaqueDelta ? drain_kernel<kCapOpaqueDelta> : drain_kernel<kCapAll>;
        hipLaunchKernelGGL(drain, dim3(drainResident), dim3(castBlock), plan.ldsWholeStack, stream, pool, plan.scene, (const FrameConstants*)dFrame, cnt,
                           dGlobals, (const SampleOut*)dSampleOut);
    }
// ... 1228 lines not shown
    if ((counters != 0) != t->instrCounters) t->InvalidateGraph();
    t->instrCounters = counters != 0;
    t->extTiming = ext_timing != 0;
    return DCRT_OK;
}

DCRT_API int dcrt_tracer_get_info(dcrt_tracer* t, dcrt_tracer_info* out)
{
    TRACER_GUARD(t);
    if (!out) return DCRT_E_INVALID_ARG;
    const CastPlan& plan = t->plan;
    const CastLaunch shipped = plan.Launch(false, false);
    out->path_pool_size = t->poolSize;
    out->scene_in_lds = t->hasScene && plan.allCached ? 1u : 0u;
    out->cached_nodes = t->hasScene ? plan.scene.cachedNodes : 0u;
    out->cached_triangles = t->hasScene ? plan.scene.cachedTris : 0u;
    out->cast_block = plan.block;
    out->traversal_stack = t->hasScene ? plan.scene.stackSize : 0u;
    out->material_generic = t->materialCaps == kCapAll ? 1u : 0u;
    out->pair_traversal = t->hasScene && plan.pair ? 1u : 0u;
    out->control_grid = t->controlGrid;
    out->material_grid = t->materialGrid;
    out->cast_grid = shipped.resident;
    out->material_lds = t->materialLds;
    out->cast_identity = plan.ident ? (plan.flat ? 2u : 1u) : 0u;
    out->stack_lds_rows = t->hasScene ? shipped.scene.stackRows : 0u;
    out->ring_rows = t->hasScene ? plan.ringRows : 0u;
    out->cast_waves_per_cu = plan.perCU * (plan.block / 64u);
    const bool cells = t->hasScene && shipped.scene.shadowRes != 0u;
    out->shadow_cells = cells ? shipped.scene.shadowRes : 0u;
    out->shadow_cell_max_leaves = cells ? t->cells.maxLeaves : 0u;
    out->shadow_cell_mean_leaves = cells ? t->cells.meanLeaves : 0.0f;
    out->shadow_inline = t->hasScene && t->FusedShadow() ? 1u : 0u;
    return DCRT_OK;
}

DCRT_API int dcrt_tracer_debug_ring_spills(dcrt_tracer* t, uint64_t* out)
{
    TRACER_GUARD(t);
    if (!out) return DCRT_E_INVALID_ARG;
    *out = 0;
    const CastLaunch shipped = t->plan.Launch(false, false);
    if (!t->hasScene || !shipped.scene.spill) return DCRT_OK;
    const size_t n = (size_t)shipped.resident * t->plan.block * shipped.scene.stackSize;
    std::vector<uint32_t> h(n);
    HIPCHECK(hipStreamSynchronize(t->stream));
    HIPCHECK(hipMemcpy(h.data(), shipped.scene.spill, n * 4, hipMemcpyDeviceToHost));
    for (const uint32_t w : h) *out += w != 0u;
    return DCRT_OK;
}

DCRT_API int dcrt_tracer_traversal_stats(dcrt_tracer* t, dcrt_traversal_stats* out)
{
    TRACER_GUARD(t);
    if (!out) return DCRT_E_INVALID_ARG;
    unsigned long long v[8];
    HIPCHECK(hipMemcpyAsync(v, t->dInstr, sizeof(v), hipMemcpyDeviceToHost, t->stream));
    HIPCHECK(hipStreamSynchronize(t->stream));
    CHECKED(t->CollectTimes());
    out->ext_node_visits = v[0]; out->ext_triangle_tests = v[1]; out->ext_blas_entries = v[2];
    out->shadow_node_visits = v[3]; out->shadow_triangle_tests = v[4]; out->shadow_blas_entries = v[5];
    out->ext_launches = t->kindLaunches[dcrt_tracer::kTimedCast];
    out->ext_kernel_ms = t->kindMs[dcrt_tracer::kTimedCast];
    out->ext_max_node_visits = v[6]; out->shadow_max_node_visits = v[7];
    out->material_launches = t->kindLaunches[dcrt_tracer::kTimedMaterial];
    out->material_kernel_ms = t->kindMs[dcrt_tracer::kTimedMaterial];
// ... 15 lines not shown
    t->pathsSkipped = 0;
    HIPCHECK(hipMemcpyAsync(t->dGlobals, &g, sizeof(Globals), hipMemcpyHostToDevice, t->stream));
    HIPCHECK(hipStreamSynchronize(t->stream));
    t->eventsUsed = 0;
    for (int k = 0; k < dcrt_tracer::kTimedKinds; ++k) {
        t->kindMs[k] = 0.0;
        t->kindLaunches[k] = 0;
    }
    return DCRT_OK;
}

DCRT_API int dcrt_tracer_synchronize(dcrt_tracer* t)
{
    TRACER_GUARD(t);
    HIPCHECK(hipStreamSynchronize(t->stream));
    return DCRT_OK;
}

DCRT_API int dcrt_tracer_get_luts(dcrt_tracer* t, dcrt_bxdf_luts* out)
{
    TRACER_GUARD(t);
    if (!out) return DCRT_E_INVALID_ARG;
    HIPCHECK(hipMemcpyAsync(out, t->dLuts, sizeof(dcrt_bxdf_luts), hipMemcpyDeviceToHost, t->stream));
    HIPCHECK(hipStreamSynchronize(t->stream));
    return DCRT_OK;
}

DCRT_API int dcrt_tracer_set_luts(dcrt_tracer* t, const dcrt_bxdf_luts* luts)
{
    TRACER_GUARD(t);
    if (!luts) return DCRT_E_INVALID_ARG;
    HIPCHECK(hipMemcpyAsync(t->dLuts, luts, sizeof(dcrt_bxdf_luts), hipMemcpyHostToDevice, t->stream));
    HIPCHECK(hipStreamSynchronize(t->stream));
    return DCRT_OK;
}

static int TraceBatch(dcrt_tracer* t, const dcrt_ray* d_rays, uint32_t n, dcrt_ray_hit* d_hits, uint32_t* d_occ, bool any, uint32_t features)
{
    if (!t->hasScene) { SetLastError("no scene uploaded"); return DCRT_E_NO_SCENE; }
    const CastPlan& plan = t->plan;
    const uint32_t grid = std::min<uint32_t>((n + plan.block - 1) / plan.block, plan.resident[0][0]);
    if (n == 0) return DCRT_OK;
    unsigned long long* instr = t->instrCounters ? t->dInstr : nullptr;
    auto kernel = any ? (instr ? batch_trace_kernel<true, true> : batch_trace_kernel<true, false>)
                      : (instr ? batch_trace_kernel<false, true> : batch_trace_kernel<false, false>);
    hipLaunchKernelGGL(kernel, dim3(grid), dim3(plan.block), plan.ldsWholeStack, t->stream, plan.scene, d_rays, n, features, d_hits, d_occ, instr);
    HIPCHECK(hipGetLastError());
    return DCRT_OK;
}

DCRT_API int dcrt_tracer_trace_rays(dcrt_tracer* t, const dcrt_ray* rays, uint32_t n, dcrt_ray_hit* out, uint32_t features)
{
    TRACER_GUARD(t);
    if ((!rays || !out) && n) return DCRT_E_INVALID_ARG;
    std::vector<void*> tmp;
    dcrt_ray* dr = nullptr; dcrt_ray_hit* dh = nullptr;
    CHECKED(DeviceAlloc(&dr, n, &tmp));
    CHECKED(DeviceAlloc(&dh, n, &tmp));
    int rc = DCRT_OK;
    if (hipMemcpyAsync(dr, rays, (size_t)n * sizeof(dcrt_ray), hipMemcpyHostToDevice, t->stream) != hipSuccess) rc = DCRT_E_HIP;
    if (rc == DCRT_OK) rc = TraceBatch(t, dr, n, dh, nullptr, false, features);
    if (rc == DCRT_OK && hipMemcpyAsync(out, dh, (size_t)n * sizeof(dcrt_ray_hit), hipMemcpyDeviceToHost, t->stream) != hipSuccess) rc = DCRT_E_HIP;
    if (hipStreamSynchronize(t->stream) != hipSuccess) rc = DCRT_E_HIP;
    FreeAll(&tmp);
    return rc;
}
// ... 264 lines not shown
}

DCRT_API int dcrt_device_math_eval(dcrt_tracer* t, int function, const float* x, uint32_t n, float* y)
{
    TRACER_GUARD(t);
    if ((!x || !y) && n) return DCRT_E_INVALID_ARG;
    std::vector<void*> tmp;
    float *dx = nullptr, *dy = nullptr;
    CHECKED(DeviceAlloc(&dx, n, &tmp));
    CHECKED(DeviceAlloc(&dy, n, &tmp));
    int rc = DCRT_OK;
    if (hipMemcpyAsync(dx, x, (size_t)n * 4, hipMemcpyHostToDevice, t->stream) != hipSuccess) rc = DCRT_E_HIP;
    if (rc == DCRT_OK && n) {
        hipLaunchKernelGGL(math_eval_kernel, dim3((n + 255) / 256), dim3(256), 0, t->stream, function, dx, n, dy);
        if (hipGetLastError() != hipSuccess) rc = DCRT_E_HIP;
    }
    if (rc == DCRT_OK && hipMemcpyAsync(y, dy, (size_t)n * 4, hipMemcpyDeviceToHost, t->stream) != hipSuccess) rc = DCRT_E_HIP;
    if (hipStreamSynchronize(t->stream) != hipSuccess) rc = DCRT_E_HIP;
    FreeAll(&tmp);
    return rc;
}

static DeviceScene LutOnlyScene(const dcrt_tracer* t)
{
    DeviceScene d{};
    d.lutBrdf = t->dLuts->brdf;
    d.lutBrdfAvg = t->dLuts->brdf_avg;
    d.lutBrdfDielectric = t->dLuts->brdf_dielectric;
    d.lutBrdfDielectricAvg = t->dLuts->brdf_dielectric_avg;
    d.lutBsdf = t->dLuts->bsdf;
    d.lutBsdfAvg = t->dLuts->bsdf_avg;
    return d;
}

DCRT_API int dcrt_device_bsdf_eval(dcrt_tracer* t, const dcrt_bsdf_probe_material* m, uint32_t features, const float* wi,
                                   const float* wo, uint32_t n, float* f, float* pdf)
{
    TRACER_GUARD(t);
    if (!m || ((!wi || !wo || !f || !pdf) && n)) return DCRT_E_INVALID_ARG;
    std::vector<void*> tmp;
    float *dwi = nullptr, *dwo = nullptr, *df = nullptr, *dpdf = nullptr;
    CHECKED(DeviceAlloc(&dwi, (size_t)n * 3, &tmp));
    CHECKED(DeviceAlloc(&dwo, (size_t)n * 3, &tmp));
    CHECKED(DeviceAlloc(&df, (size_t)n * 3, &tmp));
    CHECKED(DeviceAlloc(&dpdf, n, &tmp));
    int rc = DCRT_OK;
    if (hipMemcpyAsync(dwi, wi, (size_t)n * 12, hipMemcpyHostToDevice, t->stream) != hipSuccess) rc = DCRT_E_HIP;
    if (rc == DCRT_OK && hipMemcpyAsync(dwo, wo, (size_t)n * 12, hipMemcpyHostToDevice, t->stream) != hipSuccess) rc = DCRT_E_HIP;
    if (rc == DCRT_OK && n) {
        hipLaunchKernelGGL(bsdf_eval_kernel, dim3((n + 255) / 256), dim3(256), 0, t->stream, LutOnlyScene(t), *m, features,
                           (const float*)dwi, (const float*)dwo, n, df, dpdf);
        if (hipGetLastError() != hipSuccess) rc = DCRT_E_HIP;
    }
    if (rc == DCRT_OK && hipMemcpyAsync(f, df, (size_t)n * 12, hipMemcpyDeviceToHost, t->stream) != hipSuccess) rc = DCRT_E_HIP;
    if (rc == DCRT_OK && hipMemcpyAsync(pdf, dpdf, (size_t)n * 4, hipMemcpyDeviceToHost, t->stream) != hipSuccess) rc = DCRT_E_HIP;
    if (hipStreamSynchronize(t->stream) != hipSuccess) rc = DCRT_E_HIP;
    FreeAll(&tmp);
    return rc;
}

DCRT_API int dcrt_device_bsdf_sample(dcrt_tracer* t, const dcrt_bsdf_probe_material* m, uint32_t features, const float* wo,
                                     const float* u, uint32_t n, float* wi, float* f, float* pdf, uint32_t* delta)
{
    TRACER_GUARD(t);
    if (!m || ((!wo || !u || !wi || !f || !pdf || !delta) && n)) return DCRT_E_INVALID_ARG;
    std::vector<void*> tmp;
    float *dwo = nullptr, *du = nullptr, *dwi = nullptr, *df = nullptr, *dpdf = nullptr;
    uint32_t* ddelta = nullptr;
    CHECKED(DeviceAlloc(&dwo, (size_t)n * 3, &tmp));
    CHECKED(DeviceAlloc(&du, (size_t)n * 3, &tmp));
    CHECKED(DeviceAlloc(&dwi, (size_t)n * 3, &tmp));
    CHECKED(DeviceAlloc(&df, (size_t)n * 3, &tmp));
    CHECKED(DeviceAlloc(&dpdf, n, &tmp));
    CHECKED(DeviceAlloc(&ddelta, n, &tmp));
    int rc = DCRT_OK;
    if (hipMemcpyAsync(dwo, wo, (size_t)n * 12, hipMemcpyHostToDevice, t->stream) != hipSuccess) rc = DCRT_E_HIP;
    if (rc == DCRT_OK && hipMemcpyAsync(du, u, (size_t)n * 12, hipMemcpyHostToDevice, t->stream) != hipSuccess) rc = DCRT_E_HIP;
    if (rc == DCRT_OK && n) {
        hipLaunchKernelGGL(bsdf_sample_kernel, dim3((n + 255) / 256), dim3(256), 0, t->stream, LutOnlyScene(t), *m, features,
                           (const float*)dwo, (const float*)du, n, dwi, df, dpdf, ddelta);
        if (hipGetLastError() != hipSuccess) rc = DCRT_E_HIP;
    }
    if (rc == DCRT_OK && hipMemcpyAsync(wi, dwi, (size_t)n * 12, hipMemcpyDeviceToHost, t->stream) != hipSuccess) rc = DCRT_E_HIP;
    if (rc == DCRT_OK && hipMemcpyAsync(f, df, (size_t)n * 12, hipMemcpyDeviceToHost, t->stream) != hipSuccess) rc = DCRT_E_HIP;
    if (rc == DCRT_OK && hipMemcpyAsync(pdf, dpdf, (size_t)n * 4, hipMemcpyDeviceToHost, t->stream) != hipSuccess) rc = DCRT_E_HIP;
    if (rc == DCRT_OK && hipMemcpyAsync(delta, ddelta, (size_t)n * 4, hipMemcpyDeviceToHost, t->stream) != hipSuccess) rc = DCRT_E_HIP;
    if (hipStreamSynchronize(t->stream) != hipSuccess) rc = DCRT_E_HIP;
    FreeAll(&tmp);
    return rc;
}

}

#ifdef DCRT_WAVE_TIMELINE
extern "C" DCRT_API int dcrt_debug_wave_timeline(dcrt_tracer* t, unsigned long long* stamps, uint32_t* items)
{
    TRACER_GUARD(t);
    HIPCHECK(hipStreamSynchronize(t->stream));
    HIPCHECK(hipMemcpyFromSymbol(stamps, HIP_SYMBOL(g_waveLog), sizeof(g_waveLog)));
    HIPCHECK(hipMemcpyFromSymbol(items, HIP_SYMBOL(g_waveItems), sizeof(g_waveItems)));
    return DCRT_OK;
}
#endif

#ifdef DCRT_PHASE_CLOCKS
extern "C" DCRT_API int dcrt_debug_phase_clocks(dcrt_tracer* t, unsigned long long* out)
{
    TRACER_GUARD(t);
    HIPCHECK(hipStreamSynchronize(t->stream));
    HIPCHECK(hipMemcpyFromSymbol(out, HIP_SYMBOL(g_phaseClk), sizeof(g_phaseClk)));
    const unsigned long long zero[24] = {};
    HIPCHECK(hipMemcpyToSymbol(HIP_SYMBOL(g_phaseClk), zero, sizeof(zero)));
// ... 4 lines not shown
```

### directcomputeraytracing_amd/csrc/host/bvh_layout.cpp

```cpp
#include "bvh_layout.h"

#include <algorithm>
#include <cstring>
#include <limits>

namespace dcrt {

bool RequiredTraversalStack(const dcrt_flat_scene& s, uint32_t* out)
{
    const uint32_t n = s.bvh_node_count;
    *out = 0;
    if (n == 0) return true;
    std::vector<uint32_t> blasDepth(n, UINT32_MAX);
    std::vector<uint32_t> seen(n, UINT32_MAX);
    uint32_t walkId = 0;
    struct Item { uint32_t node, depth; };
    std::vector<Item> todo;
    auto walk = [&](uint32_t root, bool tlas, uint32_t* deepest) {
        ++walkId;
        todo.assign(1, { root, 0u });
        *deepest = 0;
        while (!todo.empty()) {
            const Item it = todo.back();
            todo.pop_back();
// ... 160 lines not shown
        const float* m = s.instance_transforms[s.instance_count + i].m;
        bool id = true;
        for (int r = 0; r < 3; ++r)
            for (int c = 0; c < 4; ++c) id = id && m[r * 4 + c] == (r == c ? 1.0f : 0.0f);
        identity[i] = id ? 1u : 0u;
    }
    return identity;
}

bool AllInstancesBitwiseIdentity(const dcrt_flat_scene& s)
{
    bool all = true;
    for (uint32_t i = 0; all && i < s.instance_count; ++i) {
        const float* m = s.instance_transforms[s.instance_count + i].m;
        for (int r = 0; r < 3; ++r)
            for (int c = 0; c < 4; ++c) {
                uint32_t bits;
                std::memcpy(&bits, &m[r * 4 + c], 4);
                all = all && bits == (r == c ? 0x3F800000u : 0u);
            }
    }
    return all;
}

bool SingleTriangleLeaves(const dcrt_flat_scene& s)
{
    for (uint32_t i = 0; i < s.bvh_node_count; ++i) {
        const uint32_t misc = s.bvh_nodes[i].misc;
        if (!(misc & 0x4u) && ((misc >> 3) & DCRT_BVHNODE_MISC_MASK_PRIMITIVE_COUNT) > 1u) return false;
    }
    return true;
}

}
```

### directcomputeraytracing_amd/csrc/host/bvh_layout.h

```cpp
#pragma once

#include <cstdint>
#include <vector>

#include "../../../include/dcrt.h"

namespace dcrt {

bool RequiredTraversalStack(const dcrt_flat_scene& s, uint32_t* out);

bool PairLayout(const dcrt_flat_scene& s, uint32_t topNodes, std::vector<dcrt_bvh_node>* out, bool quads = false);

bool EntryFreeLayout(const dcrt_flat_scene& s, std::vector<dcrt_bvh_node>* out, bool merge = true);

std::vector<uint32_t> IdentityInstances(const dcrt_flat_scene& s);

bool AllInstancesBitwiseIdentity(const dcrt_flat_scene& s);

bool SingleTriangleLeaves(const dcrt_flat_scene& s);

}
```

### directcomputeraytracing_amd/csrc/host/capi_scene.cpp

```cpp
#include <algorithm>
#include <cmath>
#include <cstdio>
#include <cstring>
#include <vector>
#include <exception>
#include <memory>
#include <string>

#include "../../../include/dcrt.h"
#include "bvh_layout.h"
#include "scene.h"
#include "shadow_cells.h"

namespace dcrt {
thread_local std::string g_lastError;
void SetLastError(const std::string& s) { g_lastError = s; }

int CheckFilterParams(const dcrt_filter_params& f)
{
    if (f.filter > DCRT_FILTER_LANCZOS) { SetLastError("unknown reconstruction filter"); return DCRT_E_INVALID_ARG; }
    if (!(f.radius >= 0.0f)) { SetLastError("filter radius is negative or NaN"); return DCRT_E_INVALID_ARG; }
    if (!(f.radius < 1073741824.0f)) { SetLastError("filter radius is 2^30 or more"); return DCRT_E_INVALID_ARG; }
    return DCRT_OK;
}
// ... 563 lines not shown
    DCRT_GUARD_END
}

DCRT_API int dcrt_shadow_cells_build(const dcrt_flat_scene* s, uint32_t resolution, dcrt_shadow_cells_info* info, uint64_t* outCells,
                                     uint32_t* outLeafWords, dcrt_bvh_node* outNodes, uint32_t nodeCapacity)
{
    if (!s || !info || !s->bvh_nodes || !s->vertices || !s->triangles || !s->instance_transforms || s->bvh_node_count == 0 ||
        resolution > dcrt::kCellMaxRes) {
        SetLastError("dcrt_shadow_cells_build: incomplete scene or resolution above the limit");
        return DCRT_E_INVALID_ARG;
    }
    *info = dcrt_shadow_cells_info{};
    std::vector<dcrt_bvh_node> flat;
    ShadowCells cells;
    if (!EntryFreeLayout(*s, &flat)) cells.reason = "no entry-free node order (a leaf with several triangles, or a malformed tree)";
    else dcrt::BuildShadowCells(flat.data(), flat.size(), *s, resolution ? resolution : dcrt::kCellDefaultRes, &cells);
    if (!cells.resolution) {
        SetLastError("no direction-cell table: " + cells.reason);
        return DCRT_OK;
    }
    if (outNodes && nodeCapacity < flat.size()) { SetLastError("dcrt_shadow_cells_build: node capacity too small"); return DCRT_E_INVALID_ARG; }
    info->resolution = cells.resolution;
    info->leaf_count = cells.leafCount;
    info->node_count = (uint32_t)flat.size();
    info->max_leaves = cells.maxLeaves;
    info->mean_leaves = cells.meanLeaves;
    info->r0 = (float)cells.r0;
    if (outCells) std::memcpy(outCells, cells.cells.data(), cells.cells.size() * sizeof(uint64_t));
    if (outLeafWords) std::memcpy(outLeafWords, cells.leafWords.data(), dcrt::kCellWords * sizeof(uint32_t));
    if (outNodes) std::memcpy(outNodes, flat.data(), flat.size() * sizeof(dcrt_bvh_node));
    return DCRT_OK;
}

DCRT_API int dcrt_shadow_cell_indices(uint32_t resolution, const float* w, uint32_t count, uint32_t* out)
{
    if (resolution == 0u || resolution > dcrt::kCellMaxRes || ((!w || !out) && count)) return DCRT_E_INVALID_ARG;
    for (uint32_t i = 0; i < count; ++i) out[i] = dcrt::ShadowCellIndex(resolution, w + (size_t)i * 3);
    return DCRT_OK;
}

}

extern "C" {

DCRT_API int dcrt_scene_get_postfx_params(const dcrt_scene* s, dcrt_postfx_params* out)
{
    if (!s || !out) return DCRT_E_INVALID_ARG;
    const dcrt::CScene& sc = s->scene;
    out->enabled = 1;
    out->auto_exposure = 1;
    out->ev100 = std::log2(sc.relativeAperture * sc.relativeAperture / sc.shutterTime * 100 / sc.iso);
    out->luminance_white = 1.0f;
    return DCRT_OK;
}

DCRT_API int dcrt_srgb_encode_thresholds(float out[255])
{
    if (!out) return DCRT_E_INVALID_ARG;
    for (int k = 0; k < 255; ++k) {
        const double c = (k + 0.5) / 255.0;
        const double lin = c <= 0.04045 ? c / 12.92 : std::pow((c + 0.055) / 1.055, 2.4);
        out[k] = (float)lin;
    }
    return DCRT_OK;
}

// ... 31 lines not shown
```

### directcomputeraytracing_amd/scene.py

```python
from __future__ import annotations

import ctypes as C
from pathlib import Path

import numpy as np

from . import _abi
from ._abi import check, f3


class Scene:

    DIRTY_LIGHTS = _abi.DIRTY_LIGHTS
    DIRTY_MATERIALS = _abi.DIRTY_MATERIALS
    DIRTY_INSTANCE_FLAGS = _abi.DIRTY_INSTANCE_FLAGS
    DIRTY_CAMERA = _abi.DIRTY_CAMERA
    DIRTY_SCENE = _abi.DIRTY_SCENE

    def __init__(self, resolution=(1920, 1080)):
        self._lib = _abi.load_library()
        h = C.c_void_p()
        check(self._lib.dcrt_scene_create(C.byref(h)), "dcrt_scene_create")
        self._h = h
        self.reset(*resolution)
# ... 155 lines not shown
        return n.value

    @property
    def resolution(self):
        w, h = C.c_uint32(), C.c_uint32()
        check(self._lib.dcrt_scene_get_resolution(self._h, C.byref(w), C.byref(h)))
        return w.value, h.value

    def bvh_info(self):
        t, n, s = C.c_uint32(), C.c_uint32(), C.c_uint32()
        check(self._lib.dcrt_scene_get_bvh_info(self._h, C.byref(t), C.byref(n), C.byref(s)))
        return {"tlas_nodes": t.value, "total_nodes": n.value, "stack_size": s.value}

    def flat(self) -> _abi.FlatScene:
        f = _abi.FlatScene()
        check(self._lib.dcrt_scene_get_flat(self._h, C.byref(f)), "GetFlat")
        return f

    def shadow_cells(self, resolution: int = 0) -> dict | None:
        f = self.flat()
        info = _abi.ShadowCellsInfo()
        check(self._lib.dcrt_shadow_cells_build(C.byref(f), int(resolution), C.byref(info), None, None, None, 0), "ShadowCellsBuild")
        if info.resolution == 0:
            return None
        R = info.resolution
        cells = np.zeros((6, R, R), np.uint64)
        words = np.zeros(128, np.uint32)
        nodes = np.zeros((info.node_count, 8), np.uint32)
        check(self._lib.dcrt_shadow_cells_build(C.byref(f), int(resolution), C.byref(info), cells.ctypes.data_as(C.POINTER(C.c_uint64)),
                                                words.ctypes.data_as(C.POINTER(C.c_uint32)),
                                                nodes.ctypes.data_as(C.POINTER(_abi.BVHNode)), info.node_count), "ShadowCellsBuild")
        return {"resolution": R, "cells": cells, "leaf_words": words, "nodes": nodes, "leaf_count": info.leaf_count,
                "mean_leaves": info.mean_leaves, "max_leaves": info.max_leaves, "r0": info.r0}

    def shadow_cell_indices(self, resolution: int, w: np.ndarray) -> np.ndarray:
        w = np.ascontiguousarray(w, np.float32).reshape(-1, 3)
        out = np.zeros(len(w), np.uint32)
        check(self._lib.dcrt_shadow_cell_indices(int(resolution), w.ctypes.data_as(C.POINTER(C.c_float)), len(w),
                                                 out.ctypes.data_as(C.POINTER(C.c_uint32))), "ShadowCellIndices")
        return out

    def postfx_params(self) -> _abi.PostFxParams:
        p = _abi.PostFxParams()
        check(self._lib.dcrt_scene_get_postfx_params(self._h, C.byref(p)), "GetPostFxParams")
        return p

    def frame_params(self, frame_seed: int = 0) -> _abi.FrameParams:
        p = _abi.FrameParams()
        check(self._lib.dcrt_scene_get_frame_params(self._h, int(frame_seed), C.byref(p)), "GetFrameParams")
        return p

    def loaded_content(self):
        nm, ni = C.c_uint32(), C.c_uint32()
        check(self._lib.dcrt_scene_get_content_counts(self._h, C.byref(nm), C.byref(ni)))
        meshes = []
        for i in range(nm.value):
            m = _abi.ObjMesh()
            check(self._lib.dcrt_scene_get_loaded_mesh(self._h, i, C.byref(m)), "GetLoadedMesh")
            nv, nt = m.vertex_count, m.triangle_count
            meshes.append({
                "vertices": np.ctypeslib.as_array(C.cast(m.vertices, C.POINTER(C.c_float)), (nv * 11,)).reshape(nv, 11).copy(),
                "indices": np.ctypeslib.as_array(m.indices, (nt * 3,)).reshape(nt, 3).copy(),
                "material_ids": np.ctypeslib.as_array(m.material_ids, (nt,)).copy()})
        instances = []
        for j in range(ni.value):
            mesh = C.c_uint32()
# ... 48 lines not shown
    return {"nodes": nodes[:count.value], "indices": reordered.reshape(-1, 3), "triangles": tri_map,
            "max_depth": depth.value, "max_stack_size": stack.value}


def load_obj_meshes(path, scene_layout: bool = True, material_index_base: int = 0) -> dict:
    lib = _abi.load_library()
    h = C.c_void_p()
    check(lib.dcrt_obj_load(str(path).encode(), _abi.OBJ_SCENE_LAYOUT if scene_layout else 0,
                            material_index_base, C.byref(h)), f"dcrt_obj_load({path})")
    try:
        n = C.c_uint32()
        check(lib.dcrt_obj_mesh_count(h, C.byref(n)))
        meshes = []
        for i in range(n.value):
            m = _abi.ObjMesh()
            check(lib.dcrt_obj_get_mesh(h, i, C.byref(m)))
            nv, nt = m.vertex_count, m.triangle_count
            verts = np.ctypeslib.as_array(C.cast(m.vertices, C.POINTER(C.c_float)), (nv * 11,)).reshape(nv, 11).copy() \
                if nv else np.zeros((0, 11), np.float32)
            idx = np.ctypeslib.as_array(m.indices, (nt * 3,)).reshape(nt, 3).copy() if nt else np.zeros((0, 3), np.uint32)
            mat = np.ctypeslib.as_array(m.material_ids, (nt,)).copy() if nt else np.zeros(0, np.uint32)
            meshes.append({"vertices": verts, "indices": idx, "material_ids": mat})
        check(lib.dcrt_obj_material_count(h, C.byref(n)))
        materials = []
        for i in range(n.value):
            mt = _abi.ObjMaterial()
            check(lib.dcrt_obj_get_material(h, i, C.byref(mt)))
            materials.append({"albedo": tuple(mt.albedo), "ior": mt.ior, "roughness": mt.roughness,
                              "opacity": mt.opacity, "albedo_texture_index": mt.albedo_texture_index,
                              "opacity_texture_index": mt.opacity_texture_index})
        return {"meshes": meshes, "materials": materials}
    finally:
        lib.dcrt_obj_free(h)
```

### directcomputeraytracing_amd/tracer.py

```python
from __future__ import annotations

import ctypes as C

import numpy as np

from . import _abi
from ._abi import check
from .scene import Scene

RAY_DTYPE = np.dtype([("origin", "<f4", 3), ("t_max", "<f4"), ("direction", "<f4", 3), ("t_min", "<f4")])
HIT_DTYPE = np.dtype([("t", "<f4"), ("u", "<f4"), ("v", "<f4"), ("triangle_id", "<u4"), ("instance_index", "<u4")])
assert RAY_DTYPE.itemsize == 32 and HIT_DTYPE.itemsize == 20

MATH_SIN, MATH_COS, MATH_EXP, MATH_ATAN = range(4)

OUTPUT_NAMES = {"path_tracing": _abi.OUTPUT_PATH_TRACING, "normal": _abi.OUTPUT_SHADING_NORMAL,
                "tangent": _abi.OUTPUT_SHADING_TANGENT, "albedo": _abi.OUTPUT_ALBEDO,
                "negative_ndotv": _abi.OUTPUT_NEGATIVE_NDOTV, "backface": _abi.OUTPUT_BACKFACE,
                "iteration_count": _abi.OUTPUT_ITERATION_COUNT}


def make_rays(origins, directions, t_min=0.0, t_max=np.inf) -> np.ndarray:
    o = np.asarray(origins, np.float32).reshape(-1, 3)
    d = np.asarray(directions, np.float32).reshape(-1, 3)
# ... 399 lines not shown

    def occluded_cells(self, rays: np.ndarray, features: int = _abi.FEATURE_DEFAULT) -> np.ndarray:
        rays = np.ascontiguousarray(rays, RAY_DTYPE)
        out = np.zeros(len(rays), np.uint32)
        check(self._lib.dcrt_tracer_trace_occlusion_cells(self._h, rays.ctypes.data_as(C.POINTER(_abi.Ray)), len(rays),
                                                          out.ctypes.data_as(C.POINTER(C.c_uint32)), int(features)),
              "TraceOcclusionCells")
        return out

    def trace_rays_device(self, d_rays: int, count: int, d_hits: int, features: int = _abi.FEATURE_DEFAULT) -> None:
        check(self._lib.dcrt_tracer_trace_rays_device(self._h, C.c_void_p(d_rays), int(count), C.c_void_p(d_hits),
                                                      int(features)), "TraceRaysDevice")

    def math_eval(self, function: int, x: np.ndarray) -> np.ndarray:
        x = np.ascontiguousarray(x, np.float32)
        y = np.empty_like(x)
        check(self._lib.dcrt_device_math_eval(self._h, int(function), x.ctypes.data_as(_abi._FP), x.size,
                                              y.ctypes.data_as(_abi._FP)), "MathEval")
        return y

    def bsdf_eval(self, material: _abi.BsdfProbeMaterial, wi: np.ndarray, wo: np.ndarray,
                  features: int = _abi.FEATURE_DEFAULT):
        wi = np.ascontiguousarray(wi, np.float32).reshape(-1, 3)
        wo = np.ascontiguousarray(wo, np.float32).reshape(-1, 3)
        if len(wi) != len(wo):
            raise ValueError("bsdf_eval: wi and wo differ in length")
        f = np.zeros_like(wi)
        pdf = np.zeros(len(wi), np.float32)
        fp = _abi._FP
        check(self._lib.dcrt_device_bsdf_eval(self._h, C.byref(material), int(features), wi.ctypes.data_as(fp),
                                              wo.ctypes.data_as(fp), len(wi), f.ctypes.data_as(fp), pdf.ctypes.data_as(fp)),
              "BsdfEval")
        return f, pdf

    def bsdf_sample(self, material: _abi.BsdfProbeMaterial, wo: np.ndarray, u: np.ndarray,
                    features: int = _abi.FEATURE_DEFAULT):
        wo = np.ascontiguousarray(wo, np.float32).reshape(-1, 3)
        u = np.ascontiguousarray(u, np.float32).reshape(-1, 3)
        if len(wo) != len(u):
            raise ValueError("bsdf_sample: wo and u differ in length")
        wi = np.zeros_like(wo)
        f = np.zeros_like(wo)
        pdf = np.zeros(len(wo), np.float32)
        delta = np.zeros(len(wo), np.uint32)
        fp = _abi._FP
        check(self._lib.dcrt_device_bsdf_sample(self._h, C.byref(material), int(features), wo.ctypes.data_as(fp),
                                                u.ctypes.data_as(fp), len(wo), wi.ctypes.data_as(fp), f.ctypes.data_as(fp),
                                                pdf.ctypes.data_as(fp), delta.ctypes.data_as(C.POINTER(C.c_uint32))),
              "BsdfSample")
        return wi, f, pdf, delta.astype(bool)


def bsdf_probe_material(type, albedo=(1.0, 1.0, 1.0), alpha=0.5, ior=1.5, two_sided=False, multiscattering=False,
                        internal_scattering=0) -> _abi.BsdfProbeMaterial:
    ior3 = (float(ior),) * 3 if np.isscalar(ior) else tuple(float(x) for x in ior)
    return _abi.BsdfProbeMaterial(int(type), (C.c_float * 3)(*albedo), (C.c_float * 3)(*ior3), float(alpha), int(two_sided),
                                  int(multiscattering), int(internal_scattering))


def denoise_default_params() -> _abi.DenoiseParams:
    p = _abi.DenoiseParams()
    check(_abi.load_library().dcrt_denoise_default_params(C.byref(p)), "DenoiseDefaultParams")
    return p


def noise_stats_dict(s: _abi.NoiseStats) -> dict:
# ... 159 lines not shown
```

### include/dcrt.h

```cpp
#ifndef DCRT_H_
#define DCRT_H_

#include <stdint.h>
#include <stddef.h>

#ifdef __cplusplus
extern "C" {
#endif

#define DCRT_API __attribute__((visibility("default")))

#define DCRT_OK              0
#define DCRT_E_INVALID_ARG  -1
#define DCRT_E_HIP          -2
#define DCRT_E_NO_SCENE     -3
#define DCRT_E_IO           -4
#define DCRT_E_LIMIT        -5
#define DCRT_E_NO_DEVICE    -6

#define DCRT_LIGHT_INDEX_INVALID        0xFFFFFFFFu
#define DCRT_LIGHT_FLAGS_POINT_LIGHT        0x1u
#define DCRT_LIGHT_FLAGS_MESH_LIGHT         0x2u
#define DCRT_LIGHT_FLAGS_DIRECTIONAL_LIGHT  0x4u
#define DCRT_LIGHT_FLAGS_ENVIRONMENT_LIGHT  0x8u
// ... 174 lines not shown
} dcrt_film_partition;

typedef struct dcrt_traversal_stats {
    uint64_t ext_node_visits, ext_triangle_tests, ext_blas_entries;
    uint64_t shadow_node_visits, shadow_triangle_tests, shadow_blas_entries;
    uint64_t ext_launches;
    double ext_kernel_ms;
    uint64_t ext_max_node_visits, shadow_max_node_visits;
    uint64_t material_launches;
    double material_kernel_ms;
    uint64_t control_launches;
    double control_kernel_ms;
} dcrt_traversal_stats;

typedef struct dcrt_tracer_info {
    uint32_t path_pool_size;
    uint32_t scene_in_lds;
    uint32_t cached_nodes, cached_triangles;
    uint32_t cast_block;
    uint32_t traversal_stack;
    uint32_t material_generic;
    uint32_t pair_traversal;
    uint32_t control_grid, material_grid;
    uint32_t cast_grid;
    uint32_t material_lds;
    uint32_t cast_identity;
    uint32_t stack_lds_rows;
    uint32_t ring_rows;
    uint32_t cast_waves_per_cu;
    uint32_t shadow_cells;
    uint32_t shadow_cell_max_leaves;
    float shadow_cell_mean_leaves;
    uint32_t shadow_inline;
} dcrt_tracer_info;

typedef struct dcrt_tracer dcrt_tracer;
typedef struct dcrt_scene dcrt_scene;

#define DCRT_ABI_VERSION 4
DCRT_API int dcrt_abi_version(void);
DCRT_API const char* dcrt_version(void);
DCRT_API const char* dcrt_last_error(void);
DCRT_API int dcrt_device_count(int* out_count);

DCRT_API int dcrt_scene_create(dcrt_scene** out_scene);
DCRT_API void dcrt_scene_destroy(dcrt_scene* scene);
DCRT_API int dcrt_scene_reset(dcrt_scene* scene, uint32_t resolution_width, uint32_t resolution_height);
DCRT_API int dcrt_scene_load_from_file(dcrt_scene* scene, const char* path);
DCRT_API int dcrt_scene_add_punctual_light(dcrt_scene* scene, const float position[3], const float euler_angles[3],
                                           const float color[3], int is_directional);
DCRT_API int dcrt_scene_set_punctual_light(dcrt_scene* scene, uint32_t index, const float position[3],
                                           const float euler_angles[3], const float color[3], int is_directional);
DCRT_API int dcrt_scene_remove_punctual_light(dcrt_scene* scene, uint32_t index);
DCRT_API int dcrt_scene_remove_environment_light(dcrt_scene* scene);
#define DCRT_DIRTY_LIGHTS          0x01u
#define DCRT_DIRTY_MATERIALS       0x02u
#define DCRT_DIRTY_INSTANCE_FLAGS  0x04u
#define DCRT_DIRTY_CAMERA          0x08u
#define DCRT_DIRTY_SCENE           0x10u
DCRT_API int dcrt_scene_acquire_dirty(dcrt_scene* scene, uint32_t* out_bits);
DCRT_API int dcrt_scene_flatten(dcrt_scene* scene);
DCRT_API int dcrt_scene_set_environment_light(dcrt_scene* scene, const float color[3],
                                              const float* cube_rgb, uint32_t cube_size);
DCRT_API int dcrt_scene_set_camera(dcrt_scene* scene, const float position[3], const float euler_angles[3]);
DCRT_API int dcrt_scene_set_lens(dcrt_scene* scene, int camera_type, float fov_x, float focal_length,
                                 float focal_distance, float relative_aperture, uint32_t blade_count,
                                 float aperture_rotation, const float film_size[2]);
DCRT_API int dcrt_scene_set_max_bounce(dcrt_scene* scene, uint32_t max_bounce);
DCRT_API int dcrt_scene_set_filter(dcrt_scene* scene, const dcrt_filter_params* filter);
DCRT_API int dcrt_scene_get_filter(const dcrt_scene* scene, dcrt_filter_params* out_filter);
DCRT_API int dcrt_scene_get_resolution(const dcrt_scene* scene, uint32_t* width, uint32_t* height);
DCRT_API int dcrt_scene_get_material_count(const dcrt_scene* scene, uint32_t* out_count);
// ... 236 lines not shown
    uint32_t active_blocks;
    uint32_t total_blocks;
} dcrt_adaptive_report;
DCRT_API int dcrt_tracer_set_adaptive(dcrt_tracer* tracer, int enable);
DCRT_API int dcrt_tracer_set_sample_blocks(dcrt_tracer* tracer, const uint32_t* blocks, uint32_t count);
DCRT_API int dcrt_tracer_get_sample_blocks(dcrt_tracer* tracer, uint32_t* out_blocks, uint32_t capacity, uint32_t* out_count);
DCRT_API int dcrt_tracer_update_sample_blocks(dcrt_tracer* tracer, float threshold, uint32_t margin, uint32_t* out_active);
DCRT_API int dcrt_tracer_sample_blocks_device(dcrt_tracer* tracer, uint32_t width, uint32_t height, const void* d_film,
                                              const void* d_half, float threshold, uint32_t margin, void* d_flags_or_null,
                                              void* d_list, uint32_t* out_count);
DCRT_API int dcrt_tracer_adaptive_timings(dcrt_tracer* tracer, float* out_mask_ms, float* out_compact_ms, float* out_fill_ms);
DCRT_API int dcrt_tracer_render_adaptive(dcrt_tracer* tracer, uint32_t first_seed, const dcrt_converge_params* params,
                                         uint32_t margin, const dcrt_filter_params* filter, dcrt_noise_stats* out_stats,
                                         int* out_converged, dcrt_adaptive_report* out_report_or_null);

DCRT_API int dcrt_write_bmp(const char* path, uint32_t width, uint32_t height, const uint8_t* rgba8);

DCRT_API int dcrt_device_math_eval(dcrt_tracer* tracer, int function, const float* x, uint32_t count, float* out_y);

typedef struct dcrt_bsdf_probe_material {
    uint32_t type;
    float albedo[3];
    float ior[3];
    float alpha;
    uint32_t two_sided, multiscattering;
    uint32_t internal_scattering_mode;
} dcrt_bsdf_probe_material;
DCRT_API int dcrt_device_bsdf_eval(dcrt_tracer* tracer, const dcrt_bsdf_probe_material* material, uint32_t features,
                                   const float* wi, const float* wo, uint32_t count, float* out_f, float* out_pdf);
DCRT_API int dcrt_device_bsdf_sample(dcrt_tracer* tracer, const dcrt_bsdf_probe_material* material, uint32_t features,
                                     const float* wo, const float* u, uint32_t count, float* out_wi, float* out_f,
                                     float* out_pdf, uint32_t* out_delta);

#ifdef __cplusplus
}
#endif

#endif
```

Measured before the change: 18120 Mrays/s.

## Precompute per-material dielectric LUT rows and per-triangle world frames for shading

Adds per-material precomputed dielectric BRDF LUT rows (optionally staged in LDS) so plastic shading does a small 1D interpolation instead of a full 3D LUT sample. Adds a per-triangle world-space frame table (normal, tangent, geometry normal, flatness flags) so flat triangles skip barycentric interpolation and the instance transform. Also skips the BSDF pdf evaluation when only delta lights exist. Costs extra memory and LDS, plus build kernels and a host instance-ownership pass. Adds probe APIs and bumps the ABI version.

Measured after the change: 19350 Mrays/s (median of 6 runs). +6.8%, better.

```diff
diff --git a/directcomputeraytracing_amd/_abi.py b/directcomputeraytracing_amd/_abi.py
--- a/directcomputeraytracing_amd/_abi.py
+++ b/directcomputeraytracing_amd/_abi.py
@@ -8,7 +8,7 @@
 LIB_PATH = PKG_DIR / "libdcrt.so"
 
 DCRT_OK = 0
-ABI_VERSION = 4
+ABI_VERSION = 5
 ERRORS = {-1: "DCRT_E_INVALID_ARG", -2: "DCRT_E_HIP", -3: "DCRT_E_NO_SCENE", -4: "DCRT_E_IO",
           -5: "DCRT_E_LIMIT", -6: "DCRT_E_NO_DEVICE"}
 LIGHT_INDEX_INVALID = 0xFFFFFFFF
@@ -166,7 +166,8 @@
                 ("material_grid", C.c_uint32), ("cast_grid", C.c_uint32), ("material_lds", C.c_uint32),
                 ("cast_identity", C.c_uint32), ("stack_lds_rows", C.c_uint32), ("ring_rows", C.c_uint32),
                 ("cast_waves_per_cu", C.c_uint32), ("shadow_cells", C.c_uint32), ("shadow_cell_max_leaves", C.c_uint32),
-                ("shadow_cell_mean_leaves", C.c_float), ("shadow_inline", C.c_uint32)]
+                ("shadow_cell_mean_leaves", C.c_float), ("shadow_inline", C.c_uint32), ("shading_tables", C.c_uint32),
+                ("dielectric_row_bytes", C.c_uint32), ("dielectric_row_lds", C.c_uint32), ("frame_table_bytes", C.c_uint32)]
 
 
 class ShadowCellsInfo(C.Structure):
@@ -356,6 +357,8 @@
     ("dcrt_write_bmp", _I, [C.c_char_p, _U, _U, C.POINTER(C.c_uint8)]),
     ("dcrt_device_math_eval", _I, [_P, _I, _FP, _U, _FP]),
     ("dcrt_device_bsdf_eval", _I, [_P, C.POINTER(BsdfProbeMaterial), _U, _FP, _FP, _U, _FP, _FP]),
+    ("dcrt_device_frame_probe", _I, [_P, C.POINTER(C.c_uint32), _U, _I, _FP]),
+    ("dcrt_flat_scene_triangle_instances", _I, [C.POINTER(FlatScene), C.POINTER(C.c_uint32), _U, C.POINTER(C.c_int)]),
     ("dcrt_device_bsdf_sample", _I, [_P, C.POINTER(BsdfProbeMaterial), _U, _FP, _FP, _U, _FP, _FP, _FP, C.POINTER(C.c_uint32)]),
 ]
 
diff --git a/directcomputeraytracing_amd/csrc/device/dbsdf.h b/directcomputeraytracing_amd/csrc/device/dbsdf.h
--- a/directcomputeraytracing_amd/csrc/device/dbsdf.h
+++ b/directcomputeraytracing_amd/csrc/device/dbsdf.h
@@ -240,10 +240,10 @@
     return wi;
 }
 
-DEV V3 isf_factor(const DeviceScene& s, float alpha, V3 albedo, float ior, uint32_t mode)
+DEV V3 isf_factor(const DeviceScene& s, float alpha, V3 albedo, float ior, uint32_t mode, const float* rows = nullptr)
 {
     if (mode == DCRT_INTERNAL_SCATTERING_IGNORE) return mk(1.0f, 1.0f, 1.0f);
-    const float avg = lut_brdf_dielectric_avg(s, alpha, ior, true);
+    const float avg = rows ? rows[130] : lut_brdf_dielectric_avg(s, alpha, ior, true);
     const float f = 1.0f - avg;
     V3 factor = mk(f, f, f);
     if (mode == DCRT_INTERNAL_SCATTERING_MULTIPLE)
@@ -300,8 +300,8 @@
         f.Eavg = lut_brdf_avg(s, it.alpha);
     }
     if (type == DCRT_MATERIAL_TYPE_PLASTIC && f.any) {
-        f.diel = lut_brdf_dielectric(s, cosO, it.alpha, it.ior.x, false);
-        f.isf = isf_factor(s, it.alpha, it.albedo, it.ior.x, it.internalScatteringMode);
+        f.diel = it.dielRows ? lut_brdf_dielectric_rows(it.dielRows, cosO) : lut_brdf_dielectric(s, cosO, it.alpha, it.ior.x, false);
+        f.isf = isf_factor(s, it.alpha, it.albedo, it.ior.x, it.internalScatteringMode, it.dielRows);
     }
     if (type == DCRT_MATERIAL_TYPE_DIELECTRIC && it.multiscattering && !(it.alpha < kAlphaThreshold))
         f.dms = dielectric_ms(s, cosO, it.alpha, it.ior.x, f.inv);
diff --git a/directcomputeraytracing_amd/csrc/device/dscene.h b/directcomputeraytracing_amd/csrc/device/dscene.h
--- a/directcomputeraytracing_amd/csrc/device/dscene.h
+++ b/directcomputeraytracing_amd/csrc/device/dscene.h
@@ -76,7 +76,21 @@
     const uint64_t* shadowCells;
     const uint32_t* shadowLeaves;
     uint32_t shadowRes;
+    const float* dielRows;
+    uint32_t ldsRows;
+    uint32_t shadingTables;
+    const float4* triFrames;
+    uint32_t ldsFrames;
 };
+
+constexpr uint32_t kTableDeltaPdf = 1u << 0;
+constexpr uint32_t kTableDielRows = 1u << 1;
+constexpr uint32_t kTableFrames = 1u << 2;
+constexpr uint32_t kTableAll = kTableDeltaPdf | kTableDielRows | kTableFrames;
+constexpr uint32_t kFrameFlatNormal = 1u, kFrameFlatTangent = 2u;
+constexpr uint32_t kDielRowFloats = 132;
+constexpr uint32_t kDielRowsMaxMaterials = 64;
+__host__ __device__ inline uint32_t diel_rows_bytes(uint32_t materials) { return 4u * kDielRowFloats * materials; }
 
 __host__ __device__ inline uint32_t material_lds_bytes(uint32_t T, uint32_t I, uint32_t M, uint32_t L)
 {
@@ -800,6 +814,42 @@
 {
     return sample_array(s.lutBrdfDielectricAvg, 16, 16, 2, alpha, (eta - 1.0f) / 2.0f, 0.0f, 1, entering ? 1u : 0u);
 }
+DEV float diel_row_value(const uint16_t* lut, const uint16_t* lutAvg, float alpha, float eta, uint32_t k)
+{
+    const float ww = (eta - 1.0f) / 2.0f;
+    const float slicePos = ww * ((float)16u - 1.0f);
+    const float fraction = slicePos - floorf(slicePos);
+    const float v = remap(16, alpha);
+    const float y = v * (float)16 - 0.5f;
+    const float fy0 = floorf(y);
+    const float fy = y - fy0;
+    if (k < 128u) {
+        const uint32_t sl = (uint32_t)(int32_t)slicePos + (k >> 6);
+        const int i = array_slice((float)sl, 32);
+        const int yy = clampi((int)fy0 + (int)((k >> 5) & 1u), 0, 16 - 1);
+        return u16tex(lut + (size_t)i * 32 * 16, (int)(k & 31u), yy, 32);
+    }
+    if (k == 128u) return fy;
+    if (k == 129u) return fraction;
+    if (k == 130u) return sample_array(lutAvg, 16, 16, 2, alpha, ww, 0.0f, 1, 1u);
+    return 0.0f;
+}
+DEV float lut_brdf_dielectric_rows(const float* r, float cosThetaO)
+{
+    const float u = remap(32, cosThetaO);
+    const float x = u * (float)32 - 0.5f;
+    const float fx0 = floorf(x);
+    const float fx = x - fx0;
+    const int x0 = clampi((int)fx0, 0, 32 - 1), x1 = clampi((int)fx0 + 1, 0, 32 - 1);
+    const float fy = r[128], fraction = r[129];
+    const float a0 = r[x0] * (1.0f - fx) + r[x1] * fx;
+    const float c0 = r[32 + x0] * (1.0f - fx) + r[32 + x1] * fx;
+    const float a = a0 * (1.0f - fy) + c0 * fy;
+    const float a1 = r[64 + x0] * (1.0f - fx) + r[64 + x1] * fx;
+    const float c1 = r[96 + x0] * (1.0f - fx) + r[96 + x1] * fx;
+    const float b = a1 * (1.0f - fy) + c1 * fy;
+    return lerp(a, b, fraction);
+}
 DEV float lut_bsdf(const DeviceScene& s, float cosThetaO, float alpha, float eta, bool entering)
 {
     return sample_array(s.lutBsdf, 32, 16, 32, cosThetaO, alpha, (eta - 1.0f) / 2.0f, 16, entering ? 16u : 0u);
@@ -868,6 +918,7 @@
     V3 position, normal, tangent, geometryNormal, ior;
     bool isTwoSided, backface, multiscattering;
     uint32_t internalScatteringMode, materialType, lightIndex, triangleIndex;
+    const float* dielRows;
 };
 
 DEV V3 bary3(V3 p0, V3 p1, V3 p2, float u, float v)
@@ -878,7 +929,28 @@
     return r1;
 }
 
-template <uint32_t CAPS = kCapAll>
+DEV V3 frame_normal(float4 a0, float4 a1, float4 a2, float u, float v)
+{
+    return normalize(bary3(mk(a0.x, a0.y, a0.z), mk(a1.x, a1.y, a1.z), mk(a2.x, a2.y, a2.z), u, v));
+}
+DEV V3 frame_tangent(float4 a0, float4 b0, float4 a1, float4 b1, float4 a2, float4 b2, float u, float v, V3 normal)
+{
+    V3 tangent = bary3(mk(a0.w, b0.x, b0.y), mk(a1.w, b1.x, b1.y), mk(a2.w, b2.x, b2.y), u, v);
+    float tl = length(tangent);
+    if (tl >= 0.000001f) {
+        tangent = tangent - normal * dot(tangent, normal);
+        tl = length(tangent);
+    }
+    if (tl < 0.000001f) {
+        tangent = cross(normal, mk(0.0f, 1.0f, 0.0f));
+        tl = length(tangent);
+        tangent = tl >= 0.000001f ? tangent : mk(1.0f, 0.0f, 0.0f);
+    }
+    return tangent / tl;
+}
+DEV V3 frame_geometry_normal(V3 p0, V3 p1, V3 p2) { return normalize(cross(p2 - p0, p1 - p0)); }
+
+template <uint32_t CAPS = kCapAll, bool FRAMES = false>
 DEV void hit_to_intersection(const DeviceScene& s, const HitRecord& h, Intersection& it)
 {
     const uint32_t inst = h.inst, tri = h.tri & 0x7FFFFFFFu;
@@ -892,20 +964,34 @@
     const float u = h.u, v = h.v;
     const V3 p0 = mk(q0.x, q0.y, q0.z), p1 = mk(q1.x, q1.y, q1.z), p2 = mk(q2.x, q2.y, q2.z);
     it.position = bary3(p0, p1, p2, u, v);
-    it.normal = normalize(bary3(mk(a0.x, a0.y, a0.z), mk(a1.x, a1.y, a1.z), mk(a2.x, a2.y, a2.z), u, v));
-    V3 tangent = bary3(mk(a0.w, b0.x, b0.y), mk(a1.w, b1.x, b1.y), mk(a2.w, b2.x, b2.y), u, v);
-    float tl = length(tangent);
-    if (tl >= 0.000001f) {
-        tangent = tangent - it.normal * dot(tangent, it.normal);
-        tl = length(tangent);
-    }
-    if (tl < 0.000001f) {
-        tangent = cross(it.normal, mk(0.0f, 1.0f, 0.0f));
-        tl = length(tangent);
-        tangent = tl >= 0.000001f ? tangent : mk(1.0f, 0.0f, 0.0f);
-    }
-    it.tangent = tangent / tl;
-    it.geometryNormal = normalize(cross(p2 - p0, p1 - p0));
+    if constexpr (!FRAMES) {
+        it.normal = frame_normal(a0, a1, a2, u, v);
+        it.tangent = frame_tangent(a0, b0, a1, b1, a2, b2, u, v, it.normal);
+        it.geometryNormal = frame_geometry_normal(p0, p1, p2);
+    } else {
+        {
+            const float4* M = s.transforms + (size_t)inst * 3;
+            const float4* F = s.triFrames;
+            uint32_t flat = 0u;
+            float4 f0 = make_float4(0.0f, 0.0f, 0.0f, 0.0f), f1 = f0, f2 = f0;
+            if (F != nullptr) {
+                F += (size_t)tri * 3;
+                f0 = F[0]; f1 = F[1]; f2 = F[2];
+                flat = ((__float_as_uint(u) | __float_as_uint(v)) & 0x80000000u) == 0u ? __float_as_uint(f0.w) : 0u;
+            }
+            if ((flat & (kFrameFlatNormal | kFrameFlatTangent)) == (kFrameFlatNormal | kFrameFlatTangent)) {
+                it.normal = mk(f0.x, f0.y, f0.z);
+                it.tangent = mk(f1.x, f1.y, f1.z);
+            } else {
+                const V3 n = frame_normal(a0, a1, a2, u, v);
+                it.tangent = normalize(mul43(frame_tangent(a0, b0, a1, b1, a2, b2, u, v, n), 0.0f, M));
+                if (flat & kFrameFlatNormal) it.normal = mk(f0.x, f0.y, f0.z);
+                else it.normal = normalize(mul43(n, 0.0f, M));
+            }
+            if (F != nullptr) it.geometryNormal = mk(f2.x, f2.y, f2.z);
+            else it.geometryNormal = normalize(mul43(frame_geometry_normal(p0, p1, p2), 0.0f, M));
+        }
+    }
     const uint32_t mid = ov != DCRT_INSTANCE_MATERIAL_OVERRIDE_NONE ? ov : __float_as_uint(q1.w);
     const dcrt_material& m = s.materials[mid];
     if constexpr ((CAPS & kCapTextures) == 0u) {
@@ -940,11 +1026,14 @@
     it.multiscattering = (m.flags & DCRT_MATERIAL_FLAG_MULTISCATTERING) != 0;
     it.internalScatteringMode = (m.flags & DCRT_MATERIAL_FLAG_INTERNAL_SCATTERING_MASK) >> DCRT_MATERIAL_FLAG_INTERNAL_SCATTERING_SHIFT;
     it.backface = (h.tri & 0x80000000u) != 0;
+    it.dielRows = s.dielRows != nullptr && (m.flags & DCRT_MATERIAL_FLAG_ROUGHNESS_TEXTURE) == 0u ? s.dielRows + (size_t)mid * kDielRowFloats : nullptr;
     const float4* M = s.transforms + (size_t)inst * 3;
     it.position = mul43(it.position, 1.0f, M);
-    it.normal = normalize(mul43(it.normal, 0.0f, M));
-    it.geometryNormal = normalize(mul43(it.geometryNormal, 0.0f, M));
-    it.tangent = normalize(mul43(it.tangent, 0.0f, M));
+    if constexpr (!FRAMES) {
+        it.normal = normalize(mul43(it.normal, 0.0f, M));
+        it.geometryNormal = normalize(mul43(it.geometryNormal, 0.0f, M));
+        it.tangent = normalize(mul43(it.tangent, 0.0f, M));
+    }
 }
 
 struct LightSample {
diff --git a/directcomputeraytracing_amd/csrc/device/kernels_impl.h b/directcomputeraytracing_amd/csrc/device/kernels_impl.h
--- a/directcomputeraytracing_amd/csrc/device/kernels_impl.h
+++ b/directcomputeraytracing_amd/csrc/device/kernels_impl.h
@@ -130,6 +130,55 @@
     g->staticFill = G ? 1u : 0u;
 }
 
+__global__ void build_diel_rows_kernel(const dcrt_material* materials, uint32_t count, const uint16_t* lut, const uint16_t* lutAvg,
+                                       float* rows)
+{
+    const uint32_t i = blockIdx.x * blockDim.x + threadIdx.x;
+    if (i >= count * kDielRowFloats) return;
+    const uint32_t m = i / kDielRowFloats, k = i % kDielRowFloats;
+    float roughness = materials[m].roughness;
+    roughness = roughness * 1.0f;
+    const float alpha = roughness * roughness;
+    rows[i] = diel_row_value(lut, lutAvg, alpha, materials[m].ior[0], k);
+}
+__global__ void probe_diel_rows_kernel(const uint16_t* lut, const uint16_t* lutAvg, float* rows, float alpha, float ior)
+{
+    const uint32_t k = blockIdx.x * blockDim.x + threadIdx.x;
+    if (k < kDielRowFloats) rows[k] = diel_row_value(lut, lutAvg, alpha, ior, k);
+}
+
+__global__ void build_tri_frames_kernel(const float4* triVerts, const float4* triShade, const float4* transforms, const uint32_t* triInstance,
+                                        uint32_t count, float4* frames)
+{
+    const uint32_t t = blockIdx.x * blockDim.x + threadIdx.x;
+    if (t >= count) return;
+    const uint32_t inst = triInstance[t];
+    float4 f0 = make_float4(0.0f, 0.0f, 0.0f, 0.0f), f1 = f0, f2 = f0;
+    if (inst != 0xFFFFFFFFu) {
+        const float4* P = triVerts + (size_t)t * 3;
+        const float4* Q = triShade + (size_t)t * 6;
+        const float4 q0 = P[0], q1 = P[1], q2 = P[2];
+        const float4 a0 = Q[0], b0 = Q[1], a1 = Q[2], b1 = Q[3], a2 = Q[4], b2 = Q[5];
+        const float4* M = transforms + (size_t)inst * 3;
+        const V3 n = frame_normal(a0, a1, a2, 0.0f, 0.0f);
+        const V3 nw = normalize(mul43(n, 0.0f, M));
+        const V3 tw = normalize(mul43(frame_tangent(a0, b0, a1, b1, a2, b2, 0.0f, 0.0f, n), 0.0f, M));
+        const V3 gw = normalize(mul43(frame_geometry_normal(mk(q0.x, q0.y, q0.z), mk(q1.x, q1.y, q1.z), mk(q2.x, q2.y, q2.z)), 0.0f, M));
+        auto same3 = [](float x0, float y0, float z0, float x1, float y1, float z1) {
+            return asu(x0) == asu(x1) && asu(y0) == asu(y1) && asu(z0) == asu(z1);
+        };
+        uint32_t flags = 0u;
+        if (same3(a0.x, a0.y, a0.z, a1.x, a1.y, a1.z) && same3(a0.x, a0.y, a0.z, a2.x, a2.y, a2.z)) flags |= kFrameFlatNormal;
+        if (same3(a0.w, b0.x, b0.y, a1.w, b1.x, b1.y) && same3(a0.w, b0.x, b0.y, a2.w, b2.x, b2.y)) flags |= kFrameFlatTangent;
+        f0 = make_float4(nw.x, nw.y, nw.z, asf(flags));
+        f1 = make_float4(tw.x, tw.y, tw.z, 0.0f);
+        f2 = make_float4(gw.x, gw.y, gw.z, 0.0f);
+    }
+    frames[(size_t)t * 3] = f0;
+    frames[(size_t)t * 3 + 1] = f1;
+    frames[(size_t)t * 3 + 2] = f2;
+}
+
 __global__ void build_tri_verts_kernel(const dcrt_vertex* vertices, const uint32_t* triangles, const uint32_t* materialIds,
                                        uint32_t count, float4* out, float4* shade)
 {
@@ -253,7 +302,7 @@
     }
 }
 
-template <uint32_t CAPS>
+template <uint32_t CAPS, bool FRAMES = false>
 __device__ __forceinline__ void shade_path(const DeviceScene& sc, const FrameConstants& fc, const HitRecord& hit, V3 dir, Rng& rng,
                                            uint32_t& flags, float4& thr, const F3& li, V3& T, V3& L, V3& lsr, bool& terminate,
                                            bool& hasShadow, V3& nO, V3& nD, float4& sO, V3& sD, float& extOpacity,
@@ -266,7 +315,7 @@
     Intersection it;
     it.lightIndex = DCRT_LIGHT_INDEX_INVALID; it.triangleIndex = 0;
     it.geometryNormal = mk(0.0f, 0.0f, 0.0f);
-    if (hasHit) hit_to_intersection<CAPS>(sc, hit, it);
+    if (hasHit) hit_to_intersection<CAPS, FRAMES>(sc, hit, it);
     DCRT_MCLK(1);
     T = mk(thr.x, thr.y, thr.z);
     L = mk(li.x, li.y, li.z);
@@ -294,7 +343,10 @@
             if (any_pos(ls.radiance) && ls.pdf > 0.0f) {
                 const V3 bsdf = evaluate_bsdf(sc, vndf, ls.wi, bf, it);
                 const float NdotWI = fabsf(dot(it.normal, ls.wi));
-                const float bsdfPdf = evaluate_bsdf_pdf(sc, vndf, ls.wi, bf, it);
+                bool wantPdf = true;
+                if constexpr ((CAPS & (kCapLightMesh | kCapLightEnv)) == 0u) wantPdf = (sc.shadingTables & kTableDeltaPdf) == 0u;
+                float bsdfPdf = 0.0f;
+                if (wantPdf) bsdfPdf = evaluate_bsdf_pdf(sc, vndf, ls.wi, bf, it);
                 const float weight = ls.isDelta ? 1.0f : power_heuristic(ls.pdf, bsdfPdf);
                 lsr = T * ls.radiance * bsdf * NdotWI * weight / ls.pdf;
                 const V3 so = offset_ray_origin(it.position, it.geometryNormal, ls.wi);
@@ -375,6 +427,12 @@
         uint32_t* ov = li + I;
         uint32_t* mt = ov + I;
         uint32_t* lt = mt + 13u * sc.ldsMaterials;
+        float* rw = (float*)(lt + 7u * sc.ldsLights);
+        for (uint32_t i = threadIdx.x; i < kDielRowFloats * sc.ldsRows; i += blockDim.x) rw[i] = sc.dielRows[i];
+        const uint32_t frameOff = material_cells_lds_offset(material_lds_bytes(T, I, sc.ldsMaterials, sc.ldsLights) + diel_rows_bytes(sc.ldsRows));
+        const uint32_t FT = sc.ldsFrames ? T : 0u;
+        float4* fr = sceneLds + (frameOff >> 4);
+        for (uint32_t i = threadIdx.x; i < 3u * FT; i += blockDim.x) fr[i] = sc.triFrames[i];
         for (uint32_t i = threadIdx.x; i < 3u * T; i += blockDim.x) tv[i] = sc.triVerts[i];
         for (uint32_t i = threadIdx.x; i < 6u * T; i += blockDim.x) ts[i] = sc.triShade[i];
         for (uint32_t i = threadIdx.x; i < 3u * I; i += blockDim.x) tf[i] = sc.transforms[i];
@@ -382,7 +440,7 @@
         for (uint32_t i = threadIdx.x; i < 13u * sc.ldsMaterials; i += blockDim.x) mt[i] = ((const uint32_t*)sc.materials)[i];
         for (uint32_t i = threadIdx.x; i < 7u * sc.ldsLights; i += blockDim.x) lt[i] = ((const uint32_t*)sc.lights)[i];
         if constexpr (FUSED) {
-            float4* cn = sceneLds + (material_cells_lds_offset(material_lds_bytes(T, I, sc.ldsMaterials, sc.ldsLights)) >> 4);
+            float4* cn = fr + 3u * FT;
             float4* ct = cn + 2u * si.nodeCount;
             uint32_t* cl = (uint32_t*)(ct + kRotTriFloat4 * T);
             for (uint32_t i = threadIdx.x; i < 2u * si.nodeCount; i += blockDim.x) cn[i] = si.nodes[i];
@@ -403,6 +461,8 @@
         sc.overrides = ov;
         sc.materials = (const dcrt_material*)mt;
         sc.lights = (const dcrt_light*)lt;
+        if (sc.ldsRows != 0u) sc.dielRows = rw;
+        if (FT != 0u) sc.triFrames = fr;
     }
     DCRT_MCLK_INIT;
     uint32_t itemsDone = 0;
@@ -479,7 +539,7 @@
         float extOpacity = 0.0f, shadowOpacity = 0.0f;
         V3 T, L, lsr;
         DCRT_MCLK(0);
-        shade_path<CAPS>(sc, fcv, hit, dir, rng, flags, thr, li, T, L, lsr, terminate, hasShadow, nO, nD, sO, sD,
+        shade_path<CAPS, SCENE_LDS == 1 && CAPS != kCapAll>(sc, fcv, hit, dir, rng, flags, thr, li, T, L, lsr, terminate, hasShadow, nO, nD, sO, sD,
                          extOpacity, shadowOpacity DCRT_MCLK_ARGS);
         DCRT_MCLK(4);
         if (fcv.features & DCRT_FEATURE_ALLOW_ANYHIT) {
@@ -1367,7 +1427,7 @@
     }
 }
 
-__device__ __forceinline__ Intersection bsdf_probe_intersection(const dcrt_bsdf_probe_material& m)
+__device__ __forceinline__ Intersection bsdf_probe_intersection(const dcrt_bsdf_probe_material& m, const float* dielRows)
 {
     Intersection it;
     it.albedo = mk(m.albedo[0], m.albedo[1], m.albedo[2]);
@@ -1384,7 +1444,22 @@
     it.materialType = m.type;
     it.lightIndex = DCRT_LIGHT_INDEX_INVALID;
     it.triangleIndex = 0;
+    it.dielRows = dielRows;
     return it;
+}
+__global__ void frame_probe_kernel(DeviceScene sc, const uint4* records, uint32_t n, float* out)
+{
+    const uint32_t i = blockIdx.x * blockDim.x + threadIdx.x;
+    if (i >= n) return;
+    const uint4 r = records[i];
+    HitRecord h;
+    h.t = 1.0f; h.u = asf(r.x); h.v = asf(r.y); h.tri = r.z; h.inst = r.w;
+    Intersection it;
+    hit_to_intersection<kCapAll, true>(sc, h, it);
+    float* o = out + (size_t)i * 9;
+    o[0] = it.normal.x; o[1] = it.normal.y; o[2] = it.normal.z;
+    o[3] = it.tangent.x; o[4] = it.tangent.y; o[5] = it.tangent.z;
+    o[6] = it.geometryNormal.x; o[7] = it.geometryNormal.y; o[8] = it.geometryNormal.z;
 }
 __global__ void bsdf_eval_kernel(DeviceScene sc, dcrt_bsdf_probe_material m, uint32_t features, const float* wi, const float* wo,
                                  uint32_t n, float* f, float* pdf)
@@ -1392,7 +1467,7 @@
     const uint32_t i = blockIdx.x * blockDim.x + threadIdx.x;
     if (i >= n) return;
     const bool vndf = (features & DCRT_FEATURE_GGX_SAMPLE_VNDF) != 0;
-    const Intersection it = bsdf_probe_intersection(m);
+    const Intersection it = bsdf_probe_intersection(m, sc.dielRows);
     const V3 a = mk(wi[3 * i], wi[3 * i + 1], wi[3 * i + 2]), b = mk(wo[3 * i], wo[3 * i + 1], wo[3 * i + 2]);
     const BsdfFrame bf = bsdf_frame(sc, b, it);
     const V3 v = evaluate_bsdf(sc, vndf, a, bf, it);
@@ -1405,7 +1480,7 @@
     const uint32_t i = blockIdx.x * blockDim.x + threadIdx.x;
     if (i >= n) return;
     const bool vndf = (features & DCRT_FEATURE_GGX_SAMPLE_VNDF) != 0;
-    const Intersection it = bsdf_probe_intersection(m);
+    const Intersection it = bsdf_probe_intersection(m, sc.dielRows);
     const V3 b = mk(wo[3 * i], wo[3 * i + 1], wo[3 * i + 2]);
     const BsdfFrame bf = bsdf_frame(sc, b, it);
     V3 w, v; float p; bool d;
diff --git a/directcomputeraytracing_amd/csrc/device/tracer.hip b/directcomputeraytracing_amd/csrc/device/tracer.hip
--- a/directcomputeraytracing_amd/csrc/device/tracer.hip
+++ b/directcomputeraytracing_amd/csrc/device/tracer.hip
@@ -254,6 +254,7 @@
     uint32_t materialLds = 16384;
     bool materialLdsPartial = true;
     uint32_t fusedShadow = 1;
+    uint32_t shadingTables = kTableAll;
 };
 ShadingKnobs ReadShadingKnobs()
 {
@@ -262,6 +263,7 @@
     k.materialLds = (uint32_t)std::max(0, EnvInt("DCRT_MATERIAL_LDS", (int)k.materialLds));
     k.materialLdsPartial = EnvFlag("DCRT_MATERIAL_LDS_PARTIAL", true);
     k.fusedShadow = (uint32_t)std::max(0, EnvInt("DCRT_FUSED_SHADOW", (int)k.fusedShadow));
+    k.shadingTables = (uint32_t)std::max(0, EnvInt("DCRT_SHADING_TABLES", (int)k.shadingTables)) & kTableAll;
     return k;
 }
 
@@ -349,6 +351,11 @@
     uint32_t materialLdsMode = 0;
     uint32_t fusedLds = 0;
     uint32_t fusedMask = 0;
+    uint32_t shadingTables = 0;
+    float* dDielRows = nullptr;
+    uint32_t dielRowsLds = 0;
+    float4* dTriFrames = nullptr;
+    uint32_t framesLds = 0;
     bool FusedShadow() const
     {
         return fusedLds != 0u && !rowProbe && plan.Cells(instrCounters, (frame.features & DCRT_FEATURE_ALLOW_ANYHIT) != 0);
@@ -475,6 +482,8 @@
     int CastOccupancy(CastFn k, size_t lds, int* out);
     void DeriveShading();
     int DeriveFusedShadow();
+    int DeriveShadingTables();
+    int BuildDielRows();
     int DeriveDrainGrid();
     int RederiveShading();
     int UpdateMaterials(const dcrt_material* materials, uint32_t count);
@@ -793,6 +802,84 @@
     return DCRT_OK;
 }
 
+static const void* MaterialKernel(uint32_t caps, uint32_t mode, bool fused)
+{
+    const bool od = caps == kCapOpaqueDelta;
+    if (fused) return od ? (const void*)material_kernel<kCapOpaqueDelta, 1, false, true> : (const void*)material_kernel<kCapAll, 1, false, true>;
+    if (mode == 1u) return od ? (const void*)material_kernel<kCapOpaqueDelta, 1> : (const void*)material_kernel<kCapAll, 1>;
+    if (mode == 2u) return od ? (const void*)material_kernel<kCapOpaqueDelta, 2> : (const void*)material_kernel<kCapAll, 2>;
+    return od ? (const void*)material_kernel<kCapOpaqueDelta, 0> : (const void*)material_kernel<kCapAll, 0>;
+}
+
+int dcrt_tracer::BuildDielRows()
+{
+    const uint32_t materialCount = (uint32_t)hostMaterials.size(), n = materialCount * kDielRowFloats;
+    hipLaunchKernelGGL(build_diel_rows_kernel, dim3((n + 255) / 256), dim3(256), 0, stream, (const dcrt_material*)dMaterials, materialCount,
+                       (const uint16_t*)dLuts->brdf_dielectric, (const uint16_t*)dLuts->brdf_dielectric_avg, dDielRows);
+    HIPCHECK(hipGetLastError());
+    return DCRT_OK;
+}
+
+int dcrt_tracer::DeriveShadingTables()
+{
+    const ShadingKnobs k = ReadShadingKnobs();
+    const uint32_t materialCount = (uint32_t)hostMaterials.size();
+    shadingTables = k.shadingTables;
+    dielRowsLds = 0;
+    framesLds = 0;
+    bool reads = false;
+    for (const dcrt_material& m : hostMaterials)
+        reads = reads || ((m.flags & DCRT_MATERIAL_FLAG_TYPE_MASK) == DCRT_MATERIAL_TYPE_PLASTIC && !(m.flags & DCRT_MATERIAL_FLAG_ROUGHNESS_TEXTURE));
+    if (!dDielRows || !reads) shadingTables &= ~kTableDielRows;
+    if (shadingTables & kTableDielRows) {
+        CHECKED(BuildDielRows());
+        if (materialLdsMode != 0u) {
+            const uint32_t rows = diel_rows_bytes(materialCount);
+            bool fits = true;
+            for (const bool fused : { false, true }) {
+                if (fused && !fusedLds) continue;
+                const void* fn = MaterialKernel(materialCaps, materialLdsMode, fused);
+                const size_t without = fused ? material_cells_lds_offset(materialLds) + fusedLds : materialLds;
+                const size_t with = fused ? material_cells_lds_offset(materialLds + rows) + fusedLds : materialLds + rows;
+                int a = 0, b = 0;
+                HIPCHECK(hipOccupancyMaxActiveBlocksPerMultiprocessor(&a, fn, (int)kMaterialBlock, without));
+                HIPCHECK(hipOccupancyMaxActiveBlocksPerMultiprocessor(&b, fn, (int)kMaterialBlock, with));
+                a = std::min(a, LdsResident(without, fn));
+                b = std::min(b, LdsResident(with, fn));
+                fits = fits && b >= a && b > 0 && with <= 65536;
+            }
+            if (fits) dielRowsLds = rows;
+        }
+    }
+    if (!dTriFrames || materialLdsMode != 1u || materialCaps == kCapAll) shadingTables &= ~kTableFrames;
+    if (shadingTables & kTableFrames) {
+        const uint32_t frames = 48u * plan.scene.triangleCount;
+        bool fits = true;
+        for (const bool fused : { false, true }) {
+            if (fused && !fusedLds) continue;
+            const void* fn = MaterialKernel(materialCaps, materialLdsMode, fused);
+            const size_t without = fused ? material_cells_lds_offset(materialLds + dielRowsLds) + fusedLds : materialLds + dielRowsLds;
+            const size_t with = material_cells_lds_offset(materialLds + dielRowsLds) + frames + (fused ? fusedLds : 0u);
+            int a = 0, b = 0;
+            HIPCHECK(hipOccupancyMaxActiveBlocksPerMultiprocessor(&a, fn, (int)kMaterialBlock, without));
+            HIPCHECK(hipOccupancyMaxActiveBlocksPerMultiprocessor(&b, fn, (int)kMaterialBlock, with));
+            a = std::min(a, LdsResident(without, fn));
+            b = std::min(b, LdsResident(with, fn));
+            fits = fits && b >= a && b > 0 && with <= 65536;
+        }
+        if (fits) framesLds = frames;
+        else shadingTables &= ~kTableFrames;
+    }
+    for (DeviceScene* d : { &plan.scene, &plan.sceneFlat, &plan.sceneRing }) {
+        d->shadingTables = shadingTables;
+        d->dielRows = (shadingTables & kTableDielRows) ? dDielRows : nullptr;
+        d->ldsRows = dielRowsLds ? materialCount : 0u;
+        d->triFrames = (shadingTables & kTableFrames) ? dTriFrames : nullptr;
+        d->ldsFrames = framesLds ? 1u : 0u;
+    }
+    return DCRT_OK;
+}
+
 int dcrt_tracer::DeriveDrainGrid()
 {
     const void* fn = materialCaps == kCapOpaqueDelta ? (const void*)drain_kernel<kCapOpaqueDelta> : (const void*)drain_kernel<kCapAll>;
@@ -808,11 +895,13 @@
     const uint32_t caps = materialCaps, mode = materialLdsMode, lds = materialLds, grid = drainResident;
     const uint32_t ldsM = plan.scene.ldsMaterials, ldsL = plan.scene.ldsLights;
     const uint32_t fused = fusedLds, mask = fusedMask;
+    const uint32_t tables = shadingTables, rowsLds = dielRowsLds + framesLds;
     DeriveShading();
     CHECKED(DeriveFusedShadow());
+    CHECKED(DeriveShadingTables());
     if (materialCaps != caps) CHECKED(DeriveDrainGrid());
     if (fusedMask != mask) newImage = true;
-    if (materialCaps != caps || materialLdsMode != mode || materialLds != lds || drainResident != grid || fusedLds != fused ||
+    if (materialCaps != caps || materialLdsMode != mode || materialLds != lds || drainResident != grid || fusedLds != fused || shadingTables != tables || dielRowsLds + framesLds != rowsLds ||
         plan.scene.ldsMaterials != ldsM || plan.scene.ldsLights != ldsL) {
         HIPCHECK(hipStreamSynchronize(stream));
         InvalidateGraph();
@@ -913,6 +1002,7 @@
     CHECKED(UploadArrays(s, &identity));
     CHECKED(PlanCast(s, k, identity));
     CHECKED(SizeGrids(k));
+    CHECKED(DeriveShadingTables());
     CHECKED(RebuildShadowCells());
     HIPCHECK(hipStreamSynchronize(stream));
     hasScene = true;
@@ -964,6 +1054,8 @@
     CHECKED(Upload(&lights, s.lights, s.light_count, shading, DCRT_MAX_LIGHT_COUNT));
     dMaterials = mats;
     dLights = lights;
+    dDielRows = nullptr;
+    if (s.material_count <= kDielRowsMaxMaterials) CHECKED(DeviceAlloc(&dDielRows, (size_t)s.material_count * kDielRowFloats, &sceneAllocs));
     dInstanceFlags = iflags;
     hostMaterials.assign(s.materials, s.materials + s.material_count);
     if (s.light_count) hostLights.assign(s.lights, s.lights + s.light_count);
@@ -976,6 +1068,17 @@
         hipLaunchKernelGGL(build_tri_verts_kernel, dim3((s.triangle_count + 255) / 256), dim3(256), 0, stream, vtx, tris, mids,
                            s.triangle_count, triVerts, triShade);
     HIPCHECK(hipGetLastError());
+    dTriFrames = nullptr;
+    std::vector<uint32_t> triInstance;
+    if (s.triangle_count && dcrt::TriangleInstances(s, &triInstance)) {
+        uint32_t* dTriInstance = nullptr;
+        CHECKED(Upload(&dTriInstance, (const uint32_t*)triInstance.data(), s.triangle_count, geometry));
+        CHECKED(DeviceAlloc(&dTriFrames, (size_t)s.triangle_count * 3, &sceneAllocs));
+        hipLaunchKernelGGL(build_tri_frames_kernel, dim3((s.triangle_count + 255) / 256), dim3(256), 0, stream, (const float4*)triVerts,
+                           (const float4*)triShade, (const float4*)xf, (const uint32_t*)dTriInstance, s.triangle_count, dTriFrames);
+        HIPCHECK(hipGetLastError());
+        HIPCHECK(hipStreamSynchronize(stream));
+    }
     std::vector<TextureDesc> descs(std::max<uint32_t>(s.texture_count, 1));
     std::vector<uint8_t> blob;
     for (uint32_t i = 0; i < s.texture_count; ++i) {
@@ -1507,7 +1610,8 @@
     const bool fused = FusedShadow();
     ShadowInline si{};
     if (fused) si = ShadowInline{ plan.sceneFlat.nodes, plan.sceneFlat.shadowCells, plan.sceneFlat.shadowLeaves, plan.sceneFlat.cachedNodes, plan.sceneFlat.shadowRes };
-    const uint32_t materialBytes = rowProbe ? 0u : fused ? material_cells_lds_offset(materialLds) + fusedLds : materialLds;
+    const uint32_t shadingBytes = framesLds ? material_cells_lds_offset(materialLds + dielRowsLds) + framesLds : materialLds + dielRowsLds;
+    const uint32_t materialBytes = rowProbe ? 0u : fused ? material_cells_lds_offset(shadingBytes) + fusedLds : shadingBytes;
     auto material = rowProbe ? material_kernel<kCapAll, 0, true>
                   : fused ? (materialCaps == kCapOpaqueDelta ? material_kernel<kCapOpaqueDelta, 1, false, true> : material_kernel<kCapAll, 1, false, true>)
                   : materialCaps == kCapOpaqueDelta
@@ -2802,6 +2906,10 @@
     out->shadow_cell_max_leaves = cells ? t->cells.maxLeaves : 0u;
     out->shadow_cell_mean_leaves = cells ? t->cells.meanLeaves : 0.0f;
     out->shadow_inline = t->hasScene && t->FusedShadow() ? 1u : 0u;
+    out->shading_tables = t->hasScene ? t->shadingTables : 0u;
+    out->dielectric_row_bytes = t->hasScene && (t->shadingTables & kTableDielRows) ? diel_rows_bytes((uint32_t)t->hostMaterials.size()) : 0u;
+    out->dielectric_row_lds = t->hasScene ? t->dielRowsLds : 0u;
+    out->frame_table_bytes = t->hasScene ? t->framesLds : 0u;
     return DCRT_OK;
 }
 
@@ -2883,6 +2991,10 @@
     if (!luts) return DCRT_E_INVALID_ARG;
     HIPCHECK(hipMemcpyAsync(t->dLuts, luts, sizeof(dcrt_bxdf_luts), hipMemcpyHostToDevice, t->stream));
     HIPCHECK(hipStreamSynchronize(t->stream));
+    if (t->hasScene && (t->shadingTables & kTableDielRows)) {
+        CHECKED(t->BuildDielRows());
+        HIPCHECK(hipStreamSynchronize(t->stream));
+    }
     return DCRT_OK;
 }
 
@@ -3213,6 +3325,19 @@
     d.lutBsdfAvg = t->dLuts->bsdf_avg;
     return d;
 }
+static int ProbeScene(dcrt_tracer* t, const dcrt_bsdf_probe_material& m, std::vector<void*>* tmp, DeviceScene* out)
+{
+    *out = LutOnlyScene(t);
+    if (!(ReadShadingKnobs().shadingTables & kTableDielRows)) return DCRT_OK;
+    float* rows = nullptr;
+    CHECKED(DeviceAlloc(&rows, kDielRowFloats, tmp));
+    hipLaunchKernelGGL(probe_diel_rows_kernel, dim3(1), dim3(256), 0, t->stream, out->lutBrdfDielectric, out->lutBrdfDielectricAvg, rows,
+                       m.alpha, m.ior[0]);
+    HIPCHECK(hipGetLastError());
+    out->dielRows = rows;
+    out->shadingTables = kTableDielRows;
+    return DCRT_OK;
+}
 
 DCRT_API int dcrt_device_bsdf_eval(dcrt_tracer* t, const dcrt_bsdf_probe_material* m, uint32_t features, const float* wi,
                                    const float* wo, uint32_t n, float* f, float* pdf)
@@ -3225,16 +3350,47 @@
     CHECKED(DeviceAlloc(&dwo, (size_t)n * 3, &tmp));
     CHECKED(DeviceAlloc(&df, (size_t)n * 3, &tmp));
     CHECKED(DeviceAlloc(&dpdf, n, &tmp));
+    DeviceScene ps;
+    if (const int prc = ProbeScene(t, *m, &tmp, &ps); prc != DCRT_OK) { FreeAll(&tmp); return prc; }
     int rc = DCRT_OK;
     if (hipMemcpyAsync(dwi, wi, (size_t)n * 12, hipMemcpyHostToDevice, t->stream) != hipSuccess) rc = DCRT_E_HIP;
     if (rc == DCRT_OK && hipMemcpyAsync(dwo, wo, (size_t)n * 12, hipMemcpyHostToDevice, t->stream) != hipSuccess) rc = DCRT_E_HIP;
     if (rc == DCRT_OK && n) {
-        hipLaunchKernelGGL(bsdf_eval_kernel, dim3((n + 255) / 256), dim3(256), 0, t->stream, LutOnlyScene(t), *m, features,
+        hipLaunchKernelGGL(bsdf_eval_kernel, dim3((n + 255) / 256), dim3(256), 0, t->stream, ps, *m, features,
                            (const float*)dwi, (const float*)dwo, n, df, dpdf);
         if (hipGetLastError() != hipSuccess) rc = DCRT_E_HIP;
     }
     if (rc == DCRT_OK && hipMemcpyAsync(f, df, (size_t)n * 12, hipMemcpyDeviceToHost, t->stream) != hipSuccess) rc = DCRT_E_HIP;
     if (rc == DCRT_OK && hipMemcpyAsync(pdf, dpdf, (size_t)n * 4, hipMemcpyDeviceToHost, t->stream) != hipSuccess) rc = DCRT_E_HIP;
+    if (hipStreamSynchronize(t->stream) != hipSuccess) rc = DCRT_E_HIP;
+    FreeAll(&tmp);
+    return rc;
+}
+
+DCRT_API int dcrt_device_frame_probe(dcrt_tracer* t, const uint32_t* records, uint32_t n, int use_table, float* out)
+{
+    TRACER_GUARD(t);
+    if ((!records || !out) && n) return DCRT_E_INVALID_ARG;
+    if (!t->hasScene || (use_table && !t->dTriFrames)) { SetLastError("no scene uploaded, or no frame table for it"); return DCRT_E_NO_SCENE; }
+    DeviceScene sc = t->plan.scene;
+    for (uint32_t i = 0; i < n; ++i) {
+        if ((records[4 * (size_t)i + 2] & 0x7FFFFFFFu) >= sc.triangleCount || records[4 * (size_t)i + 3] >= sc.instanceCount) {
+            SetLastError("frame probe: triangle or instance index out of range");
+            return DCRT_E_INVALID_ARG;
+        }
+    }
+    sc.triFrames = use_table ? t->dTriFrames : nullptr;
+    std::vector<void*> tmp;
+    uint4* drec = nullptr;
+    float* dout = nullptr;
+    int rc = DeviceAlloc(&drec, n, &tmp);
+    if (rc == DCRT_OK) rc = DeviceAlloc(&dout, (size_t)n * 9, &tmp);
+    if (rc == DCRT_OK && hipMemcpyAsync(drec, records, (size_t)n * 16, hipMemcpyHostToDevice, t->stream) != hipSuccess) rc = DCRT_E_HIP;
+    if (rc == DCRT_OK && n) {
+        hipLaunchKernelGGL(frame_probe_kernel, dim3((n + 255) / 256), dim3(256), 0, t->stream, sc, (const uint4*)drec, n, dout);
+        if (hipGetLastError() != hipSuccess) rc = DCRT_E_HIP;
+    }
+    if (rc == DCRT_OK && hipMemcpyAsync(out, dout, (size_t)n * 36, hipMemcpyDeviceToHost, t->stream) != hipSuccess) rc = DCRT_E_HIP;
     if (hipStreamSynchronize(t->stream) != hipSuccess) rc = DCRT_E_HIP;
     FreeAll(&tmp);
     return rc;
@@ -3254,11 +3410,13 @@
     CHECKED(DeviceAlloc(&df, (size_t)n * 3, &tmp));
     CHECKED(DeviceAlloc(&dpdf, n, &tmp));
     CHECKED(DeviceAlloc(&ddelta, n, &tmp));
+    DeviceScene ps;
+    if (const int prc = ProbeScene(t, *m, &tmp, &ps); prc != DCRT_OK) { FreeAll(&tmp); return prc; }
     int rc = DCRT_OK;
     if (hipMemcpyAsync(dwo, wo, (size_t)n * 12, hipMemcpyHostToDevice, t->stream) != hipSuccess) rc = DCRT_E_HIP;
     if (rc == DCRT_OK && hipMemcpyAsync(du, u, (size_t)n * 12, hipMemcpyHostToDevice, t->stream) != hipSuccess) rc = DCRT_E_HIP;
     if (rc == DCRT_OK && n) {
-        hipLaunchKernelGGL(bsdf_sample_kernel, dim3((n + 255) / 256), dim3(256), 0, t->stream, LutOnlyScene(t), *m, features,
+        hipLaunchKernelGGL(bsdf_sample_kernel, dim3((n + 255) / 256), dim3(256), 0, t->stream, ps, *m, features,
                            (const float*)dwo, (const float*)du, n, dwi, df, dpdf, ddelta);
         if (hipGetLastError() != hipSuccess) rc = DCRT_E_HIP;
     }
diff --git a/directcomputeraytracing_amd/csrc/host/bvh_layout.cpp b/directcomputeraytracing_amd/csrc/host/bvh_layout.cpp
--- a/directcomputeraytracing_amd/csrc/host/bvh_layout.cpp
+++ b/directcomputeraytracing_amd/csrc/host/bvh_layout.cpp
@@ -216,4 +216,40 @@
     return true;
 }
 
-}
+bool TriangleInstances(const dcrt_flat_scene& s, std::vector<uint32_t>* out)
+{
+    const dcrt_bvh_node* nd = s.bvh_nodes;
+    const uint32_t n = s.bvh_node_count;
+    out->assign(s.triangle_count, UINT32_MAX);
+    if (n == 0u) return false;
+    struct Item { uint32_t node, inst1; };
+    std::vector<Item> todo{{0u, 0u}};
+    size_t visits = 0;
+    while (!todo.empty()) {
+        const Item it = todo.back();
+        todo.pop_back();
+        if (it.node >= n || ++visits > (size_t)n * 4u + 64u) return false;
+        const dcrt_bvh_node& v = nd[it.node];
+        if (it.inst1 == 0u && (v.misc & 0x4u)) {
+            const uint32_t inst = (v.misc >> 3) & DCRT_BVHNODE_MISC_MASK_PRIMITIVE_COUNT;
+            if (inst >= s.instance_count) return false;
+            todo.push_back({v.right_child_or_prim_index, inst + 1u});
+        } else if (v.misc >= 4u) {
+            if (it.inst1 == 0u) return false;
+            const uint32_t count = (v.misc >> 3) & DCRT_BVHNODE_MISC_MASK_PRIMITIVE_COUNT;
+            for (uint32_t k = 0; k < count; ++k) {
+                const uint64_t t = (uint64_t)v.right_child_or_prim_index + k;
+                if (t >= s.triangle_count) return false;
+                uint32_t& owner = (*out)[(size_t)t];
+                if (owner != UINT32_MAX && owner != it.inst1 - 1u) return false;
+                owner = it.inst1 - 1u;
+            }
+        } else {
+            todo.push_back({v.right_child_or_prim_index, it.inst1});
+            todo.push_back({it.node + 1u, it.inst1});
+        }
+    }
+    return true;
+}
+
+}
diff --git a/directcomputeraytracing_amd/csrc/host/bvh_layout.h b/directcomputeraytracing_amd/csrc/host/bvh_layout.h
--- a/directcomputeraytracing_amd/csrc/host/bvh_layout.h
+++ b/directcomputeraytracing_amd/csrc/host/bvh_layout.h
@@ -19,4 +19,6 @@
 
 bool SingleTriangleLeaves(const dcrt_flat_scene& s);
 
+bool TriangleInstances(const dcrt_flat_scene& s, std::vector<uint32_t>* out);
+
 }
diff --git a/directcomputeraytracing_amd/csrc/host/capi_scene.cpp b/directcomputeraytracing_amd/csrc/host/capi_scene.cpp
--- a/directcomputeraytracing_amd/csrc/host/capi_scene.cpp
+++ b/directcomputeraytracing_amd/csrc/host/capi_scene.cpp
@@ -619,6 +619,15 @@
     return DCRT_OK;
 }
 
+DCRT_API int dcrt_flat_scene_triangle_instances(const dcrt_flat_scene* scene, uint32_t* out_instances, uint32_t capacity, int* out_single_use)
+{
+    if (!scene || !out_single_use || !scene->bvh_nodes || (!out_instances && capacity)) return DCRT_E_INVALID_ARG;
+    std::vector<uint32_t> owner;
+    *out_single_use = dcrt::TriangleInstances(*scene, &owner) ? 1 : 0;
+    for (uint32_t t = 0; t < capacity && t < owner.size(); ++t) out_instances[t] = owner[t];
+    return DCRT_OK;
+}
+
 DCRT_API int dcrt_shadow_cell_indices(uint32_t resolution, const float* w, uint32_t count, uint32_t* out)
 {
     if (resolution == 0u || resolution > dcrt::kCellMaxRes || ((!w || !out) && count)) return DCRT_E_INVALID_ARG;
diff --git a/directcomputeraytracing_amd/scene.py b/directcomputeraytracing_amd/scene.py
--- a/directcomputeraytracing_amd/scene.py
+++ b/directcomputeraytracing_amd/scene.py
@@ -211,6 +211,9 @@
                                                 nodes.ctypes.data_as(C.POINTER(_abi.BVHNode)), info.node_count), "ShadowCellsBuild")
         return {"resolution": R, "cells": cells, "leaf_words": words, "nodes": nodes, "leaf_count": info.leaf_count,
                 "mean_leaves": info.mean_leaves, "max_leaves": info.max_leaves, "r0": info.r0}
+
+    def triangle_instances(self):
+        return flat_triangle_instances(self._lib, self.flat())
 
     def shadow_cell_indices(self, resolution: int, w: np.ndarray) -> np.ndarray:
         w = np.ascontiguousarray(w, np.float32).reshape(-1, 3)
@@ -325,3 +328,11 @@
         return {"meshes": meshes, "materials": materials}
     finally:
         lib.dcrt_obj_free(h)
+
+
+def flat_triangle_instances(lib, flat):
+    owners = np.full(flat.triangle_count, 0xFFFFFFFF, np.uint32)
+    single = C.c_int(0)
+    check(lib.dcrt_flat_scene_triangle_instances(C.byref(flat), owners.ctypes.data_as(C.POINTER(C.c_uint32)), len(owners),
+                                                 C.byref(single)), "TriangleInstances")
+    return bool(single.value), owners
diff --git a/directcomputeraytracing_amd/tracer.py b/directcomputeraytracing_amd/tracer.py
--- a/directcomputeraytracing_amd/tracer.py
+++ b/directcomputeraytracing_amd/tracer.py
@@ -455,6 +455,17 @@
                                               wo.ctypes.data_as(fp), len(wi), f.ctypes.data_as(fp), pdf.ctypes.data_as(fp)),
               "BsdfEval")
         return f, pdf
+
+    def frame_probe(self, u, v, triangles, instances, use_table: bool) -> np.ndarray:
+        rec = np.empty((len(u), 4), np.uint32)
+        rec[:, 0] = np.asarray(u, np.float32).view(np.uint32)
+        rec[:, 1] = np.asarray(v, np.float32).view(np.uint32)
+        rec[:, 2] = np.asarray(triangles, np.uint32)
+        rec[:, 3] = np.asarray(instances, np.uint32)
+        out = np.zeros((len(rec), 3, 3), np.float32)
+        check(self._lib.dcrt_device_frame_probe(self._h, rec.ctypes.data_as(C.POINTER(C.c_uint32)), len(rec), int(bool(use_table)),
+                                                out.ctypes.data_as(_abi._FP)), "FrameProbe")
+        return out
 
     def bsdf_sample(self, material: _abi.BsdfProbeMaterial, wo: np.ndarray, u: np.ndarray,
                     features: int = _abi.FEATURE_DEFAULT):
diff --git a/include/dcrt.h b/include/dcrt.h
--- a/include/dcrt.h
+++ b/include/dcrt.h
@@ -230,12 +230,16 @@
     uint32_t shadow_cell_max_leaves;
     float shadow_cell_mean_leaves;
     uint32_t shadow_inline;
+    uint32_t shading_tables;
+    uint32_t dielectric_row_bytes;
+    uint32_t dielectric_row_lds;
+    uint32_t frame_table_bytes;
 } dcrt_tracer_info;
 
 typedef struct dcrt_tracer dcrt_tracer;
 typedef struct dcrt_scene dcrt_scene;
 
-#define DCRT_ABI_VERSION 4
+#define DCRT_ABI_VERSION 5
 DCRT_API int dcrt_abi_version(void);
 DCRT_API const char* dcrt_version(void);
 DCRT_API const char* dcrt_last_error(void);
@@ -538,6 +542,10 @@
                                      const float* wo, const float* u, uint32_t count, float* out_wi, float* out_f,
                                      float* out_pdf, uint32_t* out_delta);
 
+DCRT_API int dcrt_device_frame_probe(dcrt_tracer* tracer, const uint32_t* records, uint32_t count, int use_table, float* out_frames);
+
+DCRT_API int dcrt_flat_scene_triangle_instances(const dcrt_flat_scene* scene, uint32_t* out_instances, uint32_t capacity, int* out_single_use);
+
 #ifdef __cplusplus
 }
 #endif
```
